# LLNL/parelagmc

Hardware: AMD Instinct MI355X
Metric: MC samples/sec (SPDE field + Darcy QoI) at stated DoF; SpMV HBM GB/s vs roofline (higher is better)
Workload: dtype f64; 1 GPU; PDESampler cube_tet r=5, 595968 DoF (n_s=196608, n_u=399360, nnz(A)=4299072), 1 MC level, corlen 0.1, SPDE field only (BASELINE config 2), 4 x 64 realizations per step, all converged; tolerance=MINRES 300 / rel 1e-6 / abs 1e-12, solver=hybridization, batch=64, streams=4, parallelism=sample-farm x1, precond_storage=fp32

## Files before the change

include/pmc.h:

```cpp
#ifndef PMC_H_
#define PMC_H_

#include <stddef.h>
#include <stdint.h>

#ifdef __cplusplus
extern "C" {
#endif

#define PMC_OK 0
#define PMC_ERR_INVALID (-1)
#define PMC_ERR_DEVICE (-2)
#define PMC_ERR_COMM (-3)
#define PMC_ERR_INTERNAL (-4)

enum pmc_memspace { PMC_MEM_HOST = 0, PMC_MEM_DEVICE = 1 };
enum pmc_projection { PMC_PROJ_NONE = 0, PMC_PROJ_GATHER = 1, PMC_PROJ_L2 = 2 };
enum pmc_storage { PMC_STORAGE_FP32 = 0, PMC_STORAGE_FP64 = 1 };

typedef struct pmc_ctx pmc_ctx;
typedef struct pmc_sampler pmc_sampler;
typedef struct pmc_darcy pmc_darcy;

typedef struct pmc_csr {
// ... 2 lines not shown
    const int32_t* colind;
    const double* vals;
} pmc_csr;

typedef struct pmc_solver_opts {
    int32_t abi_version;
    int32_t max_iter;
    double rel_tol;
    double abs_tol;
    int32_t cheb_degree_M;
    double cheb_ratio_M;
    int32_t mg_smooth_degree;
    double mg_smooth_ratio;
    int32_t mg_coarse_degree;
    double mg_coarse_ratio;
    int32_t check_every;
    int32_t use_graph;
    double schur_scale;
    int32_t mg_coarsening;
    int32_t mini_max_rows;
    int32_t two_streams;
    int32_t precond_storage;
} pmc_solver_opts;

typedef struct pmc_stats {
    int32_t iterations;
    int32_t converged;
    double initial_norm;
    double final_norm;
    double solve_ms;
    double setup_ms;
} pmc_stats;

typedef struct pmc_sampler_level {
    int32_t n_u, n_s;
    pmc_csr M;
    pmc_csr B;
    const double* w_diag;
    pmc_csr P;
} pmc_sampler_level;

typedef struct pmc_hybrid_level {
    int32_t n_lambda, n_s;
    pmc_csr H;
    pmc_csr G;
    const double* z_diag;
    const double* w_diag;
    pmc_csr P;
} pmc_hybrid_level;

typedef struct pmc_hybrid_elements {
    int32_t n_u, n_s;
    pmc_csr M_pattern;
    const int32_t* c_ptr;
    const int32_t* c_elem;
    const double* c_val;
    pmc_csr B;
    const double* w_diag;
    pmc_csr P;
} pmc_hybrid_elements;
typedef struct pmc_hybrid_system pmc_hybrid_system;

typedef struct pmc_darcy_level {
    int32_t n_u, n_p;
    pmc_csr M_pattern;
    const int32_t* c_ptr;
    const int32_t* c_elem;
    const double* c_val;
    pmc_csr B;
    const double* rhs;
    const uint8_t* ess_mask;
    const double* ess_data;
    const double* obs;
    pmc_csr P;
} pmc_darcy_level;

int pmc_version(void);
#define PMC_ABI_VERSION 3
int pmc_abi_version(void);
int pmc_krylov_z_bytes(void);
int pmc_sampler_krylov_z_bytes(const pmc_sampler* s);
int pmc_darcy_krylov_z_bytes(const pmc_darcy* d);
uint64_t pmc_kernel_launches(void);
const char* pmc_last_error(void);
void pmc_solver_opts_default(pmc_solver_opts* opts);

int pmc_ctx_create(int device_id, pmc_ctx** out);
int pmc_ctx_create_abi(int device_id, int abi_version, pmc_ctx** out);
#ifndef PMC_NO_ABI_CHECK_MACRO
#define pmc_ctx_create(device_id, out) pmc_ctx_create_abi((device_id), PMC_ABI_VERSION, (out))
#endif
void pmc_ctx_destroy(pmc_ctx* ctx);
int pmc_ctx_synchronize(pmc_ctx* ctx);
void* pmc_ctx_stream(pmc_ctx* ctx);
int pmc_ctx_device(const pmc_ctx* ctx);
int pmc_timer_start(pmc_ctx* ctx);
int pmc_timer_stop(pmc_ctx* ctx, double* ms);

int pmc_malloc(pmc_ctx* ctx, size_t bytes, void** dptr);
int pmc_free(pmc_ctx* ctx, void* dptr);
int pmc_memcpy_h2d(pmc_ctx* ctx, void* dst, const void* src, size_t bytes);
int pmc_memcpy_d2h(pmc_ctx* ctx, void* dst, const void* src, size_t bytes);

int pmc_rng_seed(pmc_ctx* ctx, uint64_t seed, int nparts, int mypart);
int pmc_normal_fill(pmc_ctx* ctx, double mean, double sigma2, uint64_t first_sample_id, uint32_t stream,
                    int nbatch, int n, double* out, int memspace);

int pmc_sampler_create(pmc_ctx* ctx, int nlevels, int n_mc_levels, const pmc_sampler_level* levels,
                       double alpha, double matern_g, int lognormal, const pmc_solver_opts* opts,
                       pmc_sampler** out);
int pmc_sampler_create_hybrid(pmc_ctx* ctx, int nlevels, const pmc_hybrid_level* levels, double alpha, double matern_g,
                              int lognormal, const pmc_solver_opts* opts, pmc_sampler** out);
int pmc_sampler_is_hybrid(const pmc_sampler* s);
int pmc_hybrid_build(const pmc_hybrid_elements* level, double alpha, pmc_hybrid_system** out);
int pmc_hybrid_system_level(const pmc_hybrid_system* sys, pmc_hybrid_level* view);
void pmc_hybrid_system_destroy(pmc_hybrid_system* sys);
int pmc_sampler_create_hybrid_from_elements(pmc_ctx* ctx, int nlevels, const pmc_hybrid_elements* levels, double alpha,
                                            double matern_g, int lognormal, const pmc_solver_opts* opts, pmc_sampler** out);
typedef struct pmc_kl_level {
    int32_t n_s;
    const double* w_diag;
    pmc_csr P;
} pmc_kl_level;
int pmc_sampler_create_kl(pmc_ctx* ctx, int nlevels, const pmc_kl_level* levels, int nmodes, const double* evals,
                          const double* evect0, int lognormal, pmc_sampler** out);
int pmc_sampler_is_kl(const pmc_sampler* s);
typedef struct pmc_kl_eigs_opts {
    double tol;
    int32_t max_iter;
    int32_t guard;
    int32_t degree;
    uint64_t seed;
} pmc_kl_eigs_opts;
typedef struct pmc_kl_eigs_info {
    int32_t iterations;
    int32_t block_products;
    int32_t converged;
    double max_residual_rel;
    double gap_rel;
    double seconds;
} pmc_kl_eigs_info;
void pmc_kl_eigs_opts_default(pmc_kl_eigs_opts* opts);
int pmc_kl_matern_apply(pmc_ctx* ctx, int dim, int n, const double* centroids, const double* w_diag, double corlen,
                        int ncols, const double* X, double* Y);
int pmc_kl_matern_eigs(pmc_ctx* ctx, int dim, int n, const double* centroids, const double* w_diag, double corlen,
                       int nmodes, const pmc_kl_eigs_opts* opts , double* evals ,
                       double* evect0 , pmc_kl_eigs_info* info );
void pmc_sampler_destroy(pmc_sampler* s);
int pmc_sampler_set_projection(pmc_sampler* s, int level, int kind, const pmc_csr* Gt,
                               const int32_t* gather_idx, const double* inv_w_orig, int orig_size);
int pmc_sampler_num_levels(const pmc_sampler* s);
int pmc_sampler_xi_size(const pmc_sampler* s, int level);
int pmc_sampler_sample_size(const pmc_sampler* s, int level);
int64_t pmc_sampler_nnz(const pmc_sampler* s, int level);
int pmc_sampler_batch_width(const pmc_sampler* s, int level);
int pmc_sampler_true_p(const pmc_sampler* s, int level, pmc_csr* out);
int pmc_sampler_sample(pmc_sampler* s, int level, uint64_t first_sample_id, int nbatch, double* xi,
                       int memspace);
int pmc_sampler_eval(pmc_sampler* s, int level, int xi_level, int nbatch, const double* xi, double* s_out,
                     const double* init_s, int init_level, int use_init, double* embed_s_out, int memspace,
                     pmc_stats* stats);

typedef struct pmc_field_stats pmc_field_stats;
int pmc_field_stats_create(pmc_sampler* s, int level, const double* chi, int memspace, pmc_field_stats** out);
void pmc_field_stats_destroy(pmc_field_stats* fs);
int pmc_field_stats_reset(pmc_field_stats* fs);
// ... 84 lines not shown
```

parelagmc_amd/capi.py:

```python
from __future__ import annotations

import ctypes as C
import weakref
import os
from typing import Optional, Sequence

import numpy as np

_HERE = os.path.dirname(os.path.abspath(__file__))
LIB_PATH = os.path.join(_HERE, "lib", "libpmc.so")

PMC_MEM_HOST, PMC_MEM_DEVICE = 0, 1
PMC_PROJ_NONE, PMC_PROJ_GATHER, PMC_PROJ_L2 = 0, 1, 2


class PmcError(RuntimeError):
    def __init__(self, code, msg):
        super().__init__(f"libpmc error {code}: {msg}")
        self.code = code


class pmc_csr(C.Structure):
    _fields_ = [("nrows", C.c_int32), ("ncols", C.c_int32), ("rowptr", C.POINTER(C.c_int32)),
                ("colind", C.POINTER(C.c_int32)), ("vals", C.POINTER(C.c_double))]


class pmc_solver_opts(C.Structure):
    _fields_ = [("abi_version", C.c_int32), ("max_iter", C.c_int32), ("rel_tol", C.c_double), ("abs_tol", C.c_double),
                ("cheb_degree_M", C.c_int32), ("cheb_ratio_M", C.c_double),
                ("mg_smooth_degree", C.c_int32), ("mg_smooth_ratio", C.c_double),
                ("mg_coarse_degree", C.c_int32), ("mg_coarse_ratio", C.c_double), ("check_every", C.c_int32),
                ("use_graph", C.c_int32), ("schur_scale", C.c_double), ("mg_coarsening", C.c_int32), ("mini_max_rows", C.c_int32),
                ("two_streams", C.c_int32), ("precond_storage", C.c_int32)]


PMC_ABI_VERSION = 3
PMC_STORAGE_FP32, PMC_STORAGE_FP64 = 0, 1


class pmc_stats(C.Structure):
    _fields_ = [("iterations", C.c_int32), ("converged", C.c_int32), ("initial_norm", C.c_double),
                ("final_norm", C.c_double), ("solve_ms", C.c_double), ("setup_ms", C.c_double)]


class pmc_sampler_level(C.Structure):
    _fields_ = [("n_u", C.c_int32), ("n_s", C.c_int32), ("M", pmc_csr), ("B", pmc_csr),
                ("w_diag", C.POINTER(C.c_double)), ("P", pmc_csr)]


class pmc_hybrid_level(C.Structure):
    _fields_ = [("n_lambda", C.c_int32), ("n_s", C.c_int32), ("H", pmc_csr), ("G", pmc_csr),
                ("z_diag", C.POINTER(C.c_double)), ("w_diag", C.POINTER(C.c_double)), ("P", pmc_csr)]


class pmc_hybrid_elements(C.Structure):
    _fields_ = [("n_u", C.c_int32), ("n_s", C.c_int32), ("M_pattern", pmc_csr), ("c_ptr", C.POINTER(C.c_int32)),
                ("c_elem", C.POINTER(C.c_int32)), ("c_val", C.POINTER(C.c_double)), ("B", pmc_csr),
                ("w_diag", C.POINTER(C.c_double)), ("P", pmc_csr)]


class pmc_kl_level(C.Structure):
    _fields_ = [("n_s", C.c_int32), ("w_diag", C.POINTER(C.c_double)), ("P", pmc_csr)]


class pmc_kl_eigs_opts(C.Structure):
    _fields_ = [("tol", C.c_double), ("max_iter", C.c_int32), ("guard", C.c_int32), ("degree", C.c_int32),
                ("seed", C.c_uint64)]


class pmc_kl_eigs_info(C.Structure):
    _fields_ = [("iterations", C.c_int32), ("block_products", C.c_int32), ("converged", C.c_int32),
                ("max_residual_rel", C.c_double), ("gap_rel", C.c_double), ("seconds", C.c_double)]


class pmc_darcy_level(C.Structure):
    _fields_ = [("n_u", C.c_int32), ("n_p", C.c_int32), ("M_pattern", pmc_csr), ("c_ptr", C.POINTER(C.c_int32)),
                ("c_elem", C.POINTER(C.c_int32)), ("c_val", C.POINTER(C.c_double)), ("B", pmc_csr),
                ("rhs", C.POINTER(C.c_double)), ("ess_mask", C.POINTER(C.c_uint8)),
                ("ess_data", C.POINTER(C.c_double)), ("obs", C.POINTER(C.c_double)), ("P", pmc_csr)]


_VP = C.c_void_p
_DP = C.c_void_p
SYMBOLS = {
    "pmc_version": (C.c_int, []),
    "pmc_last_error": (C.c_char_p, []),
    "pmc_solver_opts_default": (None, [C.POINTER(pmc_solver_opts)]),
    "pmc_abi_version": (C.c_int, []),
    "pmc_krylov_z_bytes": (C.c_int, []),
    "pmc_sampler_krylov_z_bytes": (C.c_int, [_VP]),
    "pmc_darcy_krylov_z_bytes": (C.c_int, [_VP]),
    "pmc_kernel_launches": (C.c_uint64, []),
    "pmc_ctx_create": (C.c_int, [C.c_int, C.POINTER(_VP)]),
    "pmc_ctx_create_abi": (C.c_int, [C.c_int, C.c_int, C.POINTER(_VP)]),
    "pmc_ctx_destroy": (None, [_VP]),
    "pmc_ctx_synchronize": (C.c_int, [_VP]),
    "pmc_ctx_stream": (_VP, [_VP]),
    "pmc_ctx_device": (C.c_int, [_VP]),
    "pmc_timer_start": (C.c_int, [_VP]),
    "pmc_timer_stop": (C.c_int, [_VP, C.POINTER(C.c_double)]),
    "pmc_malloc": (C.c_int, [_VP, C.c_size_t, C.POINTER(_VP)]),
    "pmc_free": (C.c_int, [_VP, _VP]),
    "pmc_memcpy_h2d": (C.c_int, [_VP, _VP, _VP, C.c_size_t]),
    "pmc_memcpy_d2h": (C.c_int, [_VP, _VP, _VP, C.c_size_t]),
    "pmc_rng_seed": (C.c_int, [_VP, C.c_uint64, C.c_int, C.c_int]),
    "pmc_normal_fill": (C.c_int, [_VP, C.c_double, C.c_double, C.c_uint64, C.c_uint32, C.c_int, C.c_int, _DP, C.c_int]),
    "pmc_sampler_create": (C.c_int, [_VP, C.c_int, C.c_int, C.POINTER(pmc_sampler_level), C.c_double, C.c_double,
                                     C.c_int, C.POINTER(pmc_solver_opts), C.POINTER(_VP)]),
    "pmc_sampler_create_hybrid": (C.c_int, [_VP, C.c_int, C.POINTER(pmc_hybrid_level), C.c_double, C.c_double, C.c_int,
                                            C.POINTER(pmc_solver_opts), C.POINTER(_VP)]),
    "pmc_sampler_is_hybrid": (C.c_int, [_VP]),
    "pmc_sampler_create_kl": (C.c_int, [_VP, C.c_int, C.POINTER(pmc_kl_level), C.c_int, C.POINTER(C.c_double),
                                        C.POINTER(C.c_double), C.c_int, C.POINTER(_VP)]),
    "pmc_sampler_is_kl": (C.c_int, [_VP]),
    "pmc_kl_eigs_opts_default": (None, [C.POINTER(pmc_kl_eigs_opts)]),
    "pmc_kl_matern_apply": (C.c_int, [_VP, C.c_int, C.c_int, C.POINTER(C.c_double), C.POINTER(C.c_double), C.c_double, C.c_int,
                                      C.POINTER(C.c_double), C.POINTER(C.c_double)]),
    "pmc_kl_matern_eigs": (C.c_int, [_VP, C.c_int, C.c_int, C.POINTER(C.c_double), C.POINTER(C.c_double), C.c_double, C.c_int,
                                     C.POINTER(pmc_kl_eigs_opts), C.POINTER(C.c_double), C.POINTER(C.c_double),
                                     C.POINTER(pmc_kl_eigs_info)]),
    "pmc_hybrid_build": (C.c_int, [C.POINTER(pmc_hybrid_elements), C.c_double, C.POINTER(_VP)]),
    "pmc_hybrid_system_level": (C.c_int, [_VP, C.POINTER(pmc_hybrid_level)]),
    "pmc_hybrid_system_destroy": (None, [_VP]),
    "pmc_sampler_create_hybrid_from_elements": (C.c_int, [_VP, C.c_int, C.POINTER(pmc_hybrid_elements), C.c_double, C.c_double,
                                                          C.c_int, C.POINTER(pmc_solver_opts), C.POINTER(_VP)]),
    "pmc_sampler_smoother_time": (C.c_int, [_VP, C.POINTER(C.c_double), C.POINTER(C.c_int64), C.POINTER(C.c_double)]),
    "pmc_sampler_smoother_bytes": (C.c_int, [_VP, C.c_int, C.c_int, C.POINTER(C.c_double)]),
    "pmc_sampler_vcycle_info": (C.c_int, [_VP, C.c_int, C.c_int, C.POINTER(C.c_int), C.POINTER(C.c_int64)]),
    "pmc_sampler_vcycle_level": (C.c_int, [_VP, C.c_int, C.c_int, C.POINTER(C.c_int), C.POINTER(C.c_double)]),
    "pmc_sampler_vcycle_prolongator": (C.c_int, [_VP, C.c_int, C.c_int, C.POINTER(C.c_int), C.POINTER(C.c_int),
                                                 C.POINTER(C.c_int64), C.POINTER(C.c_int32), C.POINTER(C.c_int32),
                                                 C.POINTER(C.c_double)]),
    "pmc_sampler_destroy": (None, [_VP]),
    "pmc_sampler_set_projection": (C.c_int, [_VP, C.c_int, C.c_int, C.POINTER(pmc_csr), C.POINTER(C.c_int32),
                                             C.POINTER(C.c_double), C.c_int]),
    "pmc_sampler_num_levels": (C.c_int, [_VP]),
    "pmc_sampler_xi_size": (C.c_int, [_VP, C.c_int]),
    "pmc_sampler_sample_size": (C.c_int, [_VP, C.c_int]),
    "pmc_sampler_batch_width": (C.c_int, [_VP, C.c_int]),
    "pmc_darcy_batch_width": (C.c_int, [_VP, C.c_int]),
    "pmc_darcy_set_operator_timing": (C.c_int, [_VP, C.c_int]),
    "pmc_darcy_operator_time": (C.c_int, [_VP, C.POINTER(C.c_double), C.POINTER(C.c_int64), C.POINTER(C.c_double)]),
    "pmc_darcy_operator_bytes": (C.c_int, [_VP, C.c_int, C.c_int, C.POINTER(C.c_double)]),
    "pmc_darcy_poly_time": (C.c_int, [_VP, C.POINTER(C.c_double), C.POINTER(C.c_int64), C.POINTER(C.c_double)]),
    "pmc_darcy_poly_bytes": (C.c_int, [_VP, C.c_int, C.c_int, C.POINTER(C.c_double)]),
    "pmc_sampler_nnz": (C.c_int64, [_VP, C.c_int]),
    "pmc_sampler_true_p": (C.c_int, [_VP, C.c_int, C.POINTER(pmc_csr)]),
    "pmc_sampler_sample": (C.c_int, [_VP, C.c_int, C.c_uint64, C.c_int, _DP, C.c_int]),
    "pmc_sampler_eval": (C.c_int, [_VP, C.c_int, C.c_int, C.c_int, _DP, _DP, _DP, C.c_int, C.c_int, _DP, C.c_int,
                                   C.POINTER(pmc_stats)]),
    "pmc_sampler_mult": (C.c_int, [_VP, C.c_int, C.c_int, _DP, _DP, C.c_int, C.c_int, C.POINTER(pmc_stats)]),
    "pmc_sampler_apply_preconditioner": (C.c_int, [_VP, C.c_int, C.c_int, _DP, _DP, C.c_int]),
    "pmc_sampler_apply_operator": (C.c_int, [_VP, C.c_int, C.c_int, _DP, _DP, C.c_int, C.c_int, C.POINTER(C.c_double),
                                             C.POINTER(C.c_double)]),
    "pmc_sampler_set_operator_timing": (C.c_int, [_VP, C.c_int]),
    "pmc_sampler_operator_time": (C.c_int, [_VP, C.POINTER(C.c_double), C.POINTER(C.c_int64)]),
    "pmc_sampler_operator_event_overhead": (C.c_int, [_VP, C.POINTER(C.c_double)]),
    "pmc_field_stats_create": (C.c_int, [_VP, C.c_int, _DP, C.c_int, C.POINTER(_VP)]),
    "pmc_field_stats_destroy": (None, [_VP]),
    "pmc_field_stats_reset": (C.c_int, [_VP]),
    "pmc_field_stats_accumulate": (C.c_int, [_VP, C.c_int, _DP, C.c_int]),
    "pmc_field_stats_run": (C.c_int, [_VP, C.c_uint64, C.c_int64]),
    "pmc_field_stats_read": (C.c_int, [_VP, _DP, _DP, _DP, C.POINTER(C.c_int64), C.c_int]),
    "pmc_field_stats_read_sums": (C.c_int, [_VP, _DP, C.POINTER(C.c_int64), C.c_int]),
    "pmc_field_stats_chi_dot": (C.c_int, [_VP, C.c_int, _DP, _DP, C.c_int]),
    "pmc_sampler_l2_error": (C.c_int, [_VP, C.c_int, C.c_int, _DP, C.c_double, _DP, C.c_int]),
    "pmc_sampler_max_error": (C.c_int, [_VP, C.c_int, C.c_int, _DP, C.c_double, _DP, C.c_int]),
    "pmc_sampler_set_output_hierarchy": (C.c_int, [_VP, C.c_int, C.POINTER(pmc_csr), C.POINTER(C.c_double)]),
    "pmc_darcy_create": (C.c_int, [_VP, C.c_int, C.c_int, C.POINTER(pmc_darcy_level), C.c_int,
                                   C.POINTER(pmc_solver_opts), C.POINTER(_VP)]),
    "pmc_darcy_create_hybrid": (C.c_int, [_VP, C.c_int, C.c_int, C.POINTER(pmc_darcy_level), C.c_int,
                                          C.POINTER(pmc_solver_opts), C.POINTER(_VP)]),
    "pmc_darcy_destroy": (None, [_VP]),
    "pmc_darcy_num_dofs": (C.c_int, [_VP, C.c_int]),
    "pmc_darcy_num_pressure_dofs": (C.c_int, [_VP, C.c_int]),
# ... 883 lines not shown
```

parelagmc_amd/csrc/capi.hip:

```cpp
#include <dlfcn.h>

#include <atomic>
#include <cstdlib>
#include <cstring>
#include <mutex>

#include "handles.hpp"

namespace pmc {

static thread_local std::string g_last_error;
void set_last_error(const std::string& m) { g_last_error = m; }

void Ctx::activate() const { PMC_HIP(hipSetDevice(device)); }
void Ctx::phase_mark(int i) const { PMC_HIP(hipEventRecord(ev_phase[i], stream)); }
void Ctx::phase_report(pmc_stats* stats, int nb) const {
    PMC_HIP(hipEventSynchronize(ev_phase[2]));
    float setup = 0.f, solve = 0.f;
    PMC_HIP(hipEventElapsedTime(&setup, ev_phase[0], ev_phase[1]));
    PMC_HIP(hipEventElapsedTime(&solve, ev_phase[1], ev_phase[2]));
    for (int k = 0; k < nb; ++k) {
        stats[k].setup_ms = (double)setup / nb;
        stats[k].solve_ms = (double)solve / nb;
    }
}

static std::atomic<int> g_live_ctx[64];
int Ctx::contexts_on_device(int device) { return g_live_ctx[device & 63].load(); }

Lanes Ctx::lanes(bool split) {
    if (split && !stream2) {
        PMC_HIP(hipStreamCreateWithFlags(&stream2, hipStreamNonBlocking));
        PMC_HIP(hipEventCreateWithFlags(&ev_fork, hipEventDisableTiming));
        PMC_HIP(hipEventCreateWithFlags(&ev_join, hipEventDisableTiming));
    }
    return Lanes{stream, split ? stream2 : stream, ev_fork, ev_join, split};
}

template <class F>
static int guarded(F&& f) {
    try {
        f();
        return PMC_OK;
    } catch (const Error& e) {
        set_last_error(e.what());
        return e.code;
    } catch (const std::bad_alloc&) {
        set_last_error("host allocation failed");
        return PMC_ERR_INTERNAL;
    } catch (const std::exception& e) {
        set_last_error(e.what());
        return PMC_ERR_INTERNAL;
    } catch (...) {
        set_last_error("unknown exception");
        return PMC_ERR_INTERNAL;
    }
}

struct UniqueId { char internal[128]; };
struct Rccl {
    void* lib = nullptr;
    int (*GetUniqueId)(UniqueId*) = nullptr;
    int (*CommInitRank)(void**, int, UniqueId, int) = nullptr;
    int (*AllReduce)(const void*, void*, size_t, int, int, void*, hipStream_t) = nullptr;
    int (*CommDestroy)(void*) = nullptr;
    const char* (*GetErrorString)(int) = nullptr;
};
static Rccl& rccl() {
    static Rccl r;
    static std::once_flag once;
    std::call_once(once, [] {
        const char* names[] = {"librccl.so.1", "librccl.so", "/opt/rocm/lib/librccl.so.1", "/opt/rocm/lib/librccl.so"};
        for (const char* n : names) {
            r.lib = dlopen(n, RTLD_NOW | RTLD_LOCAL);
            if (r.lib) break;
        }
        if (!r.lib) return;
        r.GetUniqueId = reinterpret_cast<decltype(r.GetUniqueId)>(dlsym(r.lib, "ncclGetUniqueId"));
        r.CommInitRank = reinterpret_cast<decltype(r.CommInitRank)>(dlsym(r.lib, "ncclCommInitRank"));
        r.AllReduce = reinterpret_cast<decltype(r.AllReduce)>(dlsym(r.lib, "ncclAllReduce"));
        r.CommDestroy = reinterpret_cast<decltype(r.CommDestroy)>(dlsym(r.lib, "ncclCommDestroy"));
        r.GetErrorString = reinterpret_cast<decltype(r.GetErrorString)>(dlsym(r.lib, "ncclGetErrorString"));
    });
    if (!r.lib || !r.GetUniqueId || !r.CommInitRank || !r.AllReduce || !r.CommDestroy)
        throw Error(PMC_ERR_COMM, "RCCL (librccl.so) could not be loaded");
    return r;
}
static void rccl_check(int rc, const char* what) {
    if (rc != 0) {
        Rccl& r = rccl();
        throw Error(PMC_ERR_COMM, std::string(what) + ": " + (r.GetErrorString ? r.GetErrorString(rc) : "RCCL error"));
    }
}

}

using namespace pmc;

extern "C" {

int pmc_version(void) { return 100; }
int pmc_abi_version(void) { return PMC_ABI_VERSION; }
int pmc_krylov_z_bytes(void) { return 4; }
uint64_t pmc_kernel_launches(void) { return kernel_launch_count(); }
const char* pmc_last_error(void) { return g_last_error.c_str(); }

static void check_abi(const pmc_solver_opts& o) {
    if (o.abi_version != PMC_ABI_VERSION)
        throw Error(PMC_ERR_INVALID, "pmc_solver_opts.abi_version is " + std::to_string(o.abi_version) + ", this library has " +
                                         std::to_string(PMC_ABI_VERSION) +
                                         ": fill the struct with pmc_solver_opts_default() of the header you compile against");
}

void pmc_solver_opts_default(pmc_solver_opts* o) {
    if (!o) return;
    o->max_iter = 300;
    o->rel_tol = 1e-6;
    o->abs_tol = 1e-12;
    o->abi_version = PMC_ABI_VERSION;
    o->cheb_degree_M = 0;
    o->cheb_ratio_M = 0.0;
    o->mg_smooth_degree = 2;
    o->mg_smooth_ratio = 8.0;
    o->mg_coarse_degree = 12;
    o->mg_coarse_ratio = 100.0;
    o->check_every = 2;
    o->schur_scale = 1.0;
    o->mg_coarsening = 2;
    o->mini_max_rows = 6000;
    o->two_streams = 0;
    o->use_graph = 0;
    o->precond_storage = PMC_STORAGE_FP32;
}

#undef pmc_ctx_create
int pmc_ctx_create(int device_id, pmc_ctx** out);
int pmc_ctx_create_abi(int device_id, int abi_version, pmc_ctx** out) {
    if (abi_version != PMC_ABI_VERSION) {
        if (out) *out = nullptr;
        set_last_error("caller was compiled against PMC_ABI_VERSION " + std::to_string(abi_version) + ", this library has " +
                       std::to_string(PMC_ABI_VERSION) + " (layout of pmc_solver_opts / pmc_stats): rebuild against include/pmc.h");
        return PMC_ERR_INVALID;
    }
    return pmc_ctx_create(device_id, out);
}
int pmc_ctx_create(int device_id, pmc_ctx** out) {
    return guarded([&] {
        PMC_REQUIRE(out != nullptr, "pmc_ctx_create: out is NULL");
        *out = nullptr;
        int ndev = 0;
        hipError_t e = hipGetDeviceCount(&ndev);
        if (e != hipSuccess || ndev == 0)
            throw Error(PMC_ERR_DEVICE, "no HIP device available (libpmc has no CPU fallback)");
        PMC_REQUIRE(device_id >= 0 && device_id < ndev, "pmc_ctx_create: device id out of range");
        std::unique_ptr<pmc_ctx> c(new pmc_ctx());
        c->device = device_id;
        PMC_HIP(hipSetDevice(device_id));
        PMC_HIP(hipStreamCreateWithFlags(&c->stream, hipStreamNonBlocking));
        PMC_HIP(hipEventCreate(&c->ev0));
        PMC_HIP(hipEventCreate(&c->ev1));
        for (hipEvent_t& e : c->ev_phase) PMC_HIP(hipEventCreate(&e));
        PMC_HIP(hipHostMalloc(reinterpret_cast<void**>(&c->h_flag), sizeof(int) * 16, hipHostMallocDefault));
        PMC_HIP(hipHostMalloc(reinterpret_cast<void**>(&c->h_scal), sizeof(double) * pmc::Ctx::kHostScratch, hipHostMallocDefault));
        g_live_ctx[device_id & 63].fetch_add(1);
        *out = c.release();
    });
}

void pmc_ctx_destroy(pmc_ctx* c) {
    if (!c) return;
    g_live_ctx[c->device & 63].fetch_sub(1);
    (void)hipSetDevice(c->device);
    if (c->nccl) {
        try { rccl().CommDestroy(c->nccl); } catch (...) {}
        c->nccl = nullptr;
    }
    if (c->stream) (void)hipStreamSynchronize(c->stream);
    if (c->stream2) (void)hipStreamSynchronize(c->stream2);
    if (c->h_flag) (void)hipHostFree(c->h_flag);
    if (c->h_scal) (void)hipHostFree(c->h_scal);
    if (c->ev0) (void)hipEventDestroy(c->ev0);
    if (c->ev1) (void)hipEventDestroy(c->ev1);
    for (hipEvent_t e : c->ev_phase)
        if (e) (void)hipEventDestroy(e);
    for (hipEvent_t e : {c->ev_fork, c->ev_join})
        if (e) (void)hipEventDestroy(e);
    if (c->stream2) (void)hipStreamDestroy(c->stream2);
// ... 681 lines not shown
```

parelagmc_amd/csrc/kernels.hip:

```cpp
#include "kernels.hpp"

#include <cstddef>
#include <cstdlib>

#include <algorithm>
#include <atomic>

namespace pmc {

#ifndef PMC_KBLOCK
#define PMC_KBLOCK 256
#endif
static constexpr int kBlock = PMC_KBLOCK;
static constexpr int kWave = 64;
#ifndef PMC_LEAN_GATHER
#define PMC_LEAN_GATHER 1
#endif
static constexpr bool kLeanGather = PMC_LEAN_GATHER != 0;
#ifndef PMC_LEAN_CS
#define PMC_LEAN_CS 1
#endif
static constexpr bool kLeanCs = PMC_LEAN_CS != 0;
#ifndef PMC_EG_LATE_COEF
#define PMC_EG_LATE_COEF 1
// ... 137 lines not shown
    }
}

typedef float pmc_f4 __attribute__((ext_vector_type(4)));
__device__ __forceinline__ void pin_gathers(RawVec<float, 4> (&xr)[8]) {
    pmc_f4 q0 = {xr[0].v[0], xr[0].v[1], xr[0].v[2], xr[0].v[3]}, q1 = {xr[1].v[0], xr[1].v[1], xr[1].v[2], xr[1].v[3]};
    pmc_f4 q2 = {xr[2].v[0], xr[2].v[1], xr[2].v[2], xr[2].v[3]}, q3 = {xr[3].v[0], xr[3].v[1], xr[3].v[2], xr[3].v[3]};
    pmc_f4 q4 = {xr[4].v[0], xr[4].v[1], xr[4].v[2], xr[4].v[3]}, q5 = {xr[5].v[0], xr[5].v[1], xr[5].v[2], xr[5].v[3]};
    pmc_f4 q6 = {xr[6].v[0], xr[6].v[1], xr[6].v[2], xr[6].v[3]}, q7 = {xr[7].v[0], xr[7].v[1], xr[7].v[2], xr[7].v[3]};
    asm volatile("" : "+v"(q0), "+v"(q1), "+v"(q2), "+v"(q3), "+v"(q4), "+v"(q5), "+v"(q6), "+v"(q7));
    const pmc_f4 q[8] = {q0, q1, q2, q3, q4, q5, q6, q7};
#pragma unroll
    for (int rs = 0; rs < 8; ++rs)
#pragma unroll
        for (int c = 0; c < 4; ++c) xr[rs].v[c] = q[rs][c];
}
template <typename XT, int C, int T>
__device__ __forceinline__ void pin_gathers(RawVec<XT, C> (&)[T]) {}
template <int R, int C>
__device__ __forceinline__ void pin_block(double (&a)[R][C]) {
    if constexpr (R == 8 && C == 2)
        asm volatile("" : "+v"(a[0][0]), "+v"(a[0][1]), "+v"(a[1][0]), "+v"(a[1][1]), "+v"(a[2][0]), "+v"(a[2][1]), "+v"(a[3][0]),
                     "+v"(a[3][1]), "+v"(a[4][0]), "+v"(a[4][1]), "+v"(a[5][0]), "+v"(a[5][1]), "+v"(a[6][0]), "+v"(a[6][1]),
                     "+v"(a[7][0]), "+v"(a[7][1]));
    else if constexpr (R == 4 && C == 4)
        asm volatile("" : "+v"(a[0][0]), "+v"(a[0][1]), "+v"(a[0][2]), "+v"(a[0][3]), "+v"(a[1][0]), "+v"(a[1][1]), "+v"(a[1][2]),
                     "+v"(a[1][3]), "+v"(a[2][0]), "+v"(a[2][1]), "+v"(a[2][2]), "+v"(a[2][3]), "+v"(a[3][0]), "+v"(a[3][1]),
                     "+v"(a[3][2]), "+v"(a[3][3]));
    else if constexpr (R == 2 && C == 4)
        asm volatile("" : "+v"(a[0][0]), "+v"(a[0][1]), "+v"(a[0][2]), "+v"(a[0][3]), "+v"(a[1][0]), "+v"(a[1][1]), "+v"(a[1][2]),
                     "+v"(a[1][3]));
}

template <bool NT, int C>
__device__ __forceinline__ void load_c_nt(const double* __restrict__ p, double (&v)[C]) {
    if constexpr (NT) {
#pragma unroll
        for (int i = 0; i < C; ++i) v[i] = __builtin_nontemporal_load(p + i);
    } else {
        load_c<C>(p, v);
    }
}
template <bool NT, int C>
__device__ __forceinline__ void load_v_nt(const double* __restrict__ p, double (&v)[C]) { load_c_nt<NT, C>(p, v); }
template <bool NT, int C>
__device__ __forceinline__ void load_v_nt(const float* __restrict__ p, double (&v)[C]) {
    if constexpr (NT) {
#pragma unroll
        for (int i = 0; i < C; ++i) v[i] = (double)__builtin_nontemporal_load(p + i);
    } else {
        load_cf<C>(p, v);
    }
}
template <bool NT, int C>
__device__ __forceinline__ void store_c_nt(double* __restrict__ p, const double (&v)[C]) {
    if constexpr (NT) {
#pragma unroll
        for (int i = 0; i < C; ++i) __builtin_nontemporal_store(v[i], p + i);
    } else {
        store_c<C>(p, v);
    }
}

template <bool NT, int C>
__device__ __forceinline__ void store_c_stream(double* __restrict__ p, const double (&v)[C]) {
    if constexpr (NT) {
#pragma unroll
        for (int i = 0; i < C; ++i) __builtin_nontemporal_store(v[i], p + i);
    } else {
        store_c<C>(p, v);
    }
}
template <bool NT>
__device__ __forceinline__ int load_stream(const int* __restrict__ p) {
    if constexpr (NT) return __builtin_nontemporal_load(p);
    else return *p;
}
template <bool NT>
__device__ __forceinline__ double load_stream(const double* __restrict__ p) {
    if constexpr (NT) return __builtin_nontemporal_load(p);
    else return *p;
}

template <bool NT, int C>
__device__ __forceinline__ void store_v_stream(double* __restrict__ p, const double (&v)[C]) { store_c_stream<NT, C>(p, v); }
template <bool NT, int C>
__device__ __forceinline__ void store_v_stream(float* __restrict__ p, const double (&v)[C]) {
    if constexpr (NT) {
#pragma unroll
        for (int i = 0; i < C; ++i) __builtin_nontemporal_store((float)v[i], p + i);
    } else {
        store_v<C>(p, v);
    }
}

template <int NB>
__device__ __forceinline__ void load_row(const double* __restrict__ p, double (&v)[NB]) {
    if constexpr (NB == 1) {
        v[0] = p[0];
    } else {
        const double2* q = reinterpret_cast<const double2*>(p);
#pragma unroll
        for (int i = 0; i < NB / 2; ++i) {
            double2 t = q[i];
            v[2 * i] = t.x;
            v[2 * i + 1] = t.y;
        }
    }
}
template <int NB>
__device__ __forceinline__ void store_row(double* __restrict__ p, const double (&v)[NB]) {
    if constexpr (NB == 1) {
        p[0] = v[0];
    } else {
        double2* q = reinterpret_cast<double2*>(p);
#pragma unroll
        for (int i = 0; i < NB / 2; ++i) q[i] = make_double2(v[2 * i], v[2 * i + 1]);
    }
}

__device__ __forceinline__ int vblock() { return (int)(blockIdx.z * gridDim.x + blockIdx.x); }
__device__ __forceinline__ int vgrid() { return (int)(gridDim.z * gridDim.x); }

template <int NB>
__device__ __forceinline__ void reduce_cols_store(double (&p)[Lay<NB>::C], double* __restrict__ partial, int LD = NB) {
    constexpr int C = Lay<NB>::C, T = Lay<NB>::T;
    __shared__ double lds[kBlock / kWave][NB];
#pragma unroll
    for (int c = 0; c < C; ++c) {
        double v = p[c];
#pragma unroll
        for (int off = kWave / 2; off >= T; off >>= 1) v += __shfl_xor(v, off, kWave);
        p[c] = v;
    }
    const int lane = threadIdx.x & (kWave - 1), wave = threadIdx.x / kWave;
    if (lane < T) {
#pragma unroll
        for (int c = 0; c < C; ++c) lds[wave][lane * C + c] = p[c];
    }
    __syncthreads();
    if (threadIdx.x < NB) {
        double s = 0.0;
#pragma unroll
        for (int w = 0; w < kBlock / kWave; ++w) s += lds[w][threadIdx.x];
        partial[(size_t)vblock() * LD + threadIdx.x] = s;
    }
}

__device__ __forceinline__ void reduce_cols_store_wide(const double (&p)[4], double* __restrict__ partial, int W) {
    __shared__ double lds[kBlock * 4];
#pragma unroll
    for (int c = 0; c < 4; ++c) lds[threadIdx.x * 4 + c] = p[c];
    __syncthreads();
    if ((int)threadIdx.x < W) {
        double s = 0.0;
        for (int m = threadIdx.x; m < kBlock * 4; m += W) s += lds[m];
        partial[(size_t)blockIdx.x * W + threadIdx.x] = s;
    }
}
template <int NB>
__device__ __forceinline__ void reduce_flat_store(double (&p)[Lay<NB>::C], double* __restrict__ partial, int W) {
    if constexpr (NB == kGroup) {
        if (W > NB) {
            reduce_cols_store_wide(p, partial, W);
            return;
        }
// ... 107 lines not shown
                        for (int c = 0; c < C; ++c) pdot[c] = fma((double)xr[rs].v[c], acc[rs][c], pdot[c]);
                } else if (xlast) {
#pragma unroll
                    for (int rs = 0; rs < T; ++rs)
#pragma unroll
                        for (int c = 0; c < C; ++c) xlast[rs][c] = (double)xr[rs].v[c];
                }
            }
            cj = cn;
            vj = vn;
        }
        return;
    }
    for (int j = 0; j < width; ++j, slot += kWave) {
        int cn = cj;
        double vn = vj;
        if (j + 1 < width) {
            cn = load_stream<NT>(cols + slot + kWave);
            if constexpr (!BV) vn = load_stream<NT>(vals + slot + kWave);
        }
        int cc[T];
        double aa[T];
#pragma unroll
        for (int rs = 0; rs < T; ++rs) {
            const int src = rs * G + g;
            cc[rs] = (T == 1) ? cj : __shfl(cj, src, kWave);
            if constexpr (!BV) aa[rs] = (T == 1) ? vj : __shfl(vj, src, kWave);
        }
        double xv[T][C];
        double av[T][C];
        double sv[T][C];
        if constexpr (T > 1) __builtin_amdgcn_sched_barrier(0);
#pragma unroll
        for (int rs = 0; rs < T; ++rs) {
            load_v<C>(x + (size_t)cc[rs] * LD + t * C, xv[rs]);
            if constexpr (CS) load_c<C>(cs + (size_t)cc[rs] * LD + t * C, sv[rs]);
            if constexpr (BV) load_bv<BV, C>(vals, (size_t)(slot - lane + rs * G + g) * LD + t * C, av[rs]);
        }
        if constexpr (T > 1) __builtin_amdgcn_sched_barrier(0);
#pragma unroll
        for (int rs = 0; rs < T; ++rs) {
#pragma unroll
            for (int c = 0; c < C; ++c) {
                if constexpr (CS) xv[rs][c] *= sv[rs][c];
                if constexpr (BV) acc[rs][c] = fma(av[rs][c], xv[rs][c], acc[rs][c]);
                else acc[rs][c] = fma(aa[rs], xv[rs][c], acc[rs][c]);
            }
        }
        if (xlast && j + 1 == width) {
#pragma unroll
            for (int rs = 0; rs < T; ++rs)
#pragma unroll
                for (int c = 0; c < C; ++c) xlast[rs][c] = xv[rs][c];
        }
        cj = cn;
        vj = vn;
    }
}

template <int NB, int BV, typename XT = double>
__device__ __forceinline__ void sell_row_product(const int* __restrict__ slice_off, const int* __restrict__ cols,
                                                 const double* __restrict__ vals, const XT* __restrict__ x,
                                                 int slice, int lane, int LD, double (&acc)[Lay<NB>::T][Lay<NB>::C]) {
    const int off = slice_off[slice];
    const int width = (slice_off[slice + 1] - off) >> 6;
    sell_row_range<NB, BV, false, true, false, XT>(cols, vals, x, nullptr, off, width, lane, LD, acc);
}

struct SliceWalk {
    int begin, end, stride;
};
__device__ __forceinline__ SliceWalk slice_walk(int nslices) {
    constexpr int WPB = kBlock / kWave;
    const int nblk = vgrid(), bid = vblock(), wave = threadIdx.x / kWave;
    if (nblk < 8) return SliceWalk{bid * WPB + wave, nslices, nblk * WPB};
    const int xcd = bid % 8, idx = bid / 8;
    const int nb_x = nblk / 8 + (xcd < nblk % 8 ? 1 : 0);
    const int per = (nslices + 7) / 8;
    const int lo = min(xcd * per, nslices), hi = min(lo + per, nslices);
    return SliceWalk{lo + idx * WPB + wave, hi, nb_x * WPB};
}

template <int NB, int BV, int MODE, bool DOT, int TAG, bool NT = false, bool R8 = false, bool DL = false, typename XT = double,
          typename YT = double>
__global__ __launch_bounds__(kBlock, (NB >= 32 && BV == 0 && sizeof(XT) == 4 ? 3 : 1)) void sell_spmm_kernel(int nrows, int nslices, const int* __restrict__ slice_off,
                                                           const int* __restrict__ sched,
                                                           const int* __restrict__ cols,
                                                           const double* __restrict__ vals,
                                                           const XT* __restrict__ x, typename ident<YT>::type* __restrict__ y,
                                                           const double* __restrict__ r,
                                                           const typename ident<XT>::type* __restrict__ dot_with,
                                                           double* __restrict__ partial, int ld) {
    static_assert(!R8 || (MODE == 2 && !DOT), "fused restriction goes with the residual");
    static_assert(sizeof(YT) == 8 || (MODE == 0 && !DOT && !NT), "fp32 result: plain products only");
    const int LD = row_ld<NB>(ld);
    {
        const int c0 = col0<NB>();
        x += c0;
        y += c0;
        if constexpr (BV) vals = shift_bv<BV>(vals, c0);
        if constexpr (MODE == 2) r += c0;
        if constexpr (DOT && !DL) dot_with += c0;
        if constexpr (DOT || R8) partial += c0;
    }
    static_assert(!DL || (DOT && !BV && Lay<NB>::T > 1), "diagonal-last serves the fused <x, Ax> of shared-value operators");
    constexpr int C = Lay<NB>::C, T = Lay<NB>::T, G = Lay<NB>::G;
    const int lane = threadIdx.x & (kWave - 1);
    const int g = lane / T, t = lane % T;
    double p[C];
#pragma unroll
    for (int c = 0; c < C; ++c) p[c] = 0.0;
    const SliceWalk sw = slice_walk(nslices);
    for (int si = sw.begin; si < sw.end; si += sw.stride) {
        const int slice = sched ? sched[si] : si;
        double acc[T][C];
        constexpr bool LEAN_DL = DL && lean_range<NB>();
        double xd[DL && !LEAN_DL ? T : 1][C];
        if constexpr (LEAN_DL) {
            const int off = slice_off[slice];
            sell_row_range<NB, false, false, true, NT, XT>(cols, vals, x, nullptr, off, (slice_off[slice + 1] - off) >> 6,
                                                             lane, LD, acc, nullptr, p);
        } else if constexpr (DL) {
            const int off = slice_off[slice];
            sell_row_range<NB, false, false, true, NT, XT>(cols, vals, x, nullptr, off, (slice_off[slice + 1] - off) >> 6,
                                                             lane, LD, acc, xd);
        } else if constexpr (NT) {
            const int off = slice_off[slice];
            sell_row_range<NB, BV, false, true, true, XT>(cols, vals, x, nullptr, off, (slice_off[slice + 1] - off) >> 6, lane, LD, acc);
        } else {
            sell_row_product<NB, BV, XT>(slice_off, cols, vals, x, slice, lane, LD, acc);
        }
#pragma unroll
        for (int rs = 0; rs < T; ++rs) {
            const int row = slice * kWave + rs * G + g;
            if (row < nrows) {
                const size_t at = (size_t)row * LD + t * C;
                if constexpr (MODE == 1) {
                    double old[C];
                    load_c<C>(y + at, old);
#pragma unroll
                    for (int c = 0; c < C; ++c) acc[rs][c] += old[c];
                } else if constexpr (MODE == 2) {
                    double rv[C];
                    load_c<C>(r + at, rv);
#pragma unroll
                    for (int c = 0; c < C; ++c) acc[rs][c] = rv[c] - acc[rs][c];
                }
                if constexpr (sizeof(YT) == 8) store_c_stream<NT, C>(y + at, acc[rs]);
                else store_v<C>(y + at, acc[rs]);
                if constexpr (LEAN_DL) {
                } else if constexpr (DL) {
#pragma unroll
                    for (int c = 0; c < C; ++c) p[c] = fma(xd[rs][c], acc[rs][c], p[c]);
                } else if constexpr (DOT) {
                    double w[C];
                    load_v<C>(dot_with + at, w);
#pragma unroll
                    for (int c = 0; c < C; ++c) p[c] = fma(w[c], acc[rs][c], p[c]);
                }
            } else if constexpr (R8) {
#pragma unroll
                for (int c = 0; c < C; ++c) acc[rs][c] = 0.0;
            }
            if constexpr (R8) {
                double s[C];
#pragma unroll
                for (int c = 0; c < C; ++c) {
                    double v = acc[rs][c];
                    v += __shfl_xor(v, T, kWave);
                    v += __shfl_xor(v, 2 * T, kWave);
                    v += __shfl_xor(v, 4 * T, kWave);
                    s[c] = v;
                }
                if ((g & 7) == 0 && row < nrows) store_c<C>(partial + (size_t)(row >> 3) * LD + t * C, s);
            }
        }
    }
    if constexpr (DOT) reduce_cols_store<NB>(p, partial, LD);
}

template <int NB, int BV, bool DOT, typename OT = double>
__global__ __launch_bounds__(kBlock) void sell_cheb_kernel(int nrows, int nslices, const int* __restrict__ slice_off,
                                                           const int* __restrict__ sched,
                                                           const int* __restrict__ cols,
                                                           const double* __restrict__ vals,
                                                           const double* __restrict__ dinv,
                                                           const double* __restrict__ r,
                                                           const double* __restrict__ xin, double* __restrict__ d,
                                                           OT* __restrict__ xout, double a, double b,
                                                           double* __restrict__ partial, int ld) {
    constexpr int C = Lay<NB>::C, T = Lay<NB>::T, G = Lay<NB>::G;
    const int LD = row_ld<NB>(ld);
    {
        const int c0 = col0<NB>();
        r += c0; xin += c0; d += c0; xout += c0;
        if constexpr (BV) { vals = shift_bv<BV>(vals, c0); dinv += c0; }
        if constexpr (DOT) partial += c0;
    }
    const int lane = threadIdx.x & (kWave - 1);
    const int g = lane / T, t = lane % T;
    double p[C];
#pragma unroll
    for (int c = 0; c < C; ++c) p[c] = 0.0;
    const SliceWalk sw = slice_walk(nslices);
    for (int si = sw.begin; si < sw.end; si += sw.stride) {
        const int slice = sched ? sched[si] : si;
        double acc[T][C];
        sell_row_product<NB, BV>(slice_off, cols, vals, xin, slice, lane, LD, acc);
#pragma unroll
        for (int rs = 0; rs < T; ++rs) {
            const int row = slice * kWave + rs * G + g;
            if (row >= nrows) continue;
            const size_t at = (size_t)row * LD + t * C;
            double rv[C], dv[C], xv[C], di[C];
            load_c<C>(r + at, rv);
            load_c<C>(xin + at, xv);
            if (a != 0.0) {
                load_c<C>(d + at, dv);
            } else {
#pragma unroll
                for (int c = 0; c < C; ++c) dv[c] = 0.0;
            }
            if constexpr (BV) {
                load_c<C>(dinv + at, di);
            } else {
                const double s = dinv[row];
#pragma unroll
                for (int c = 0; c < C; ++c) di[c] = s;
            }
#pragma unroll
            for (int c = 0; c < C; ++c) {
// ... 808 lines not shown
    load_c<C>(w1 + e, w1v);
    load_c<C>(x + e, xv);
#pragma unroll
    for (int c = 0; c < C; ++c) {
        w0v[c] = c0[k0 + c] * uv[c] + c1[k0 + c] * w0v[c] + c2[k0 + c] * w1v[c];
        xv[c] += c3[k0 + c] * w0v[c];
    }
    store_c<C>(w0 + e, w0v);
    store_c<C>(x + e, xv);
}

template <int NB, bool BV, bool DOT>
__global__ __launch_bounds__(kBlock) void cheb_first_kernel(size_t nflat, const double* __restrict__ dinv,
                                                            const double* __restrict__ r, double* __restrict__ d,
                                                            double* __restrict__ x, double b,
                                                            double* __restrict__ partial, int ld) {
    constexpr int C = Lay<NB>::C;
    const int W = row_ld<NB>(ld);
    double p[C];
#pragma unroll
    for (int c = 0; c < C; ++c) p[c] = 0.0;
    for (size_t i = (size_t)blockIdx.x * kBlock + threadIdx.x; i < nflat; i += (size_t)gridDim.x * kBlock) {
        const size_t e = i * C;
        double rv[C], di[C], xv[C];
        load_c<C>(r + e, rv);
        if constexpr (BV) {
            load_c<C>(dinv + e, di);
        } else {
            const double s = dinv[e / W];
#pragma unroll
            for (int c = 0; c < C; ++c) di[c] = s;
        }
#pragma unroll
        for (int c = 0; c < C; ++c) {
            xv[c] = b * di[c] * rv[c];
            if constexpr (DOT) p[c] = fma(rv[c], xv[c], p[c]);
        }
        store_c<C>(d + e, xv);
        store_c<C>(x + e, xv);
    }
    if constexpr (DOT) reduce_flat_store<NB>(p, partial, W);
}

template <int NB, typename BT = double>
__global__ __launch_bounds__(kBlock) void dot_kernel(size_t nflat, const double* __restrict__ a,
                                                     const BT* __restrict__ b, double* __restrict__ partial, int ld) {
    constexpr int C = Lay<NB>::C;
    double p[C];
#pragma unroll
    for (int c = 0; c < C; ++c) p[c] = 0.0;
    for (size_t i = (size_t)blockIdx.x * kBlock + threadIdx.x; i < nflat; i += (size_t)gridDim.x * kBlock) {
        double av[C], bv[C];
        load_c<C>(a + i * C, av);
        load_v<C>(b + i * C, bv);
#pragma unroll
        for (int c = 0; c < C; ++c) p[c] = fma(av[c], bv[c], p[c]);
    }
    reduce_flat_store<NB>(p, partial, row_ld<NB>(ld));
}

template <int NB, bool DOT, typename OT>
__global__ __launch_bounds__(kBlock) void convert_dot_kernel(size_t nflat, const double* __restrict__ in,
                                                             OT* __restrict__ out, const double* __restrict__ r,
                                                             double* __restrict__ partial, int ld) {
    constexpr int C = Lay<NB>::C;
    double p[C];
#pragma unroll
    for (int c = 0; c < C; ++c) p[c] = 0.0;
    for (size_t i = (size_t)blockIdx.x * kBlock + threadIdx.x; i < nflat; i += (size_t)gridDim.x * kBlock) {
        double v[C];
        load_c<C>(in + i * C, v);
        round_to<OT>(v);
        if constexpr (DOT) {
            double rv[C];
            load_c<C>(r + i * C, rv);
#pragma unroll
            for (int c = 0; c < C; ++c) p[c] = fma(rv[c], v[c], p[c]);
        }
        store_v<C>(out + i * C, v);
    }
    if constexpr (DOT) reduce_flat_store<NB>(p, partial, row_ld<NB>(ld));
}

template <int NB, bool NT = false>
__global__ __launch_bounds__(kBlock) void lincomb3_kernel(size_t nflat, const double* __restrict__ c0,
                                                          const double* __restrict__ a, const double* __restrict__ c1,
                                                          const double* __restrict__ b, const double* __restrict__ c2,
                                                          double* __restrict__ y, int ld, float* __restrict__ y32 = nullptr) {
    constexpr int C = Lay<NB>::C;
    const size_t i = (size_t)blockIdx.x * kBlock + threadIdx.x;
    if (i >= nflat) return;
    const size_t e = i * C;
    const int k0 = (int)(e % row_ld<NB>(ld));
    double av[C], bv[C], yv[C];
    load_c_nt<NT, C>(a + e, av);
    load_c_nt<NT, C>(b + e, bv);
    load_c_nt<NT, C>(y + e, yv);
#pragma unroll
    for (int c = 0; c < C; ++c) yv[c] = c0[k0 + c] * av[c] + c1[k0 + c] * bv[c] + c2[k0 + c] * yv[c];
    store_c<C>(y + e, yv);
    if (y32) store_v<C>(y32 + e, yv);
}

template <int NB, bool NT, typename UT>
__global__ __launch_bounds__(kBlock) void minres_wx_kernel(size_t nflat, const double* __restrict__ c0,
                                                           const UT* __restrict__ u, const double* __restrict__ c1,
                                                           double* __restrict__ w0, const double* __restrict__ c2,
                                                           const double* __restrict__ w1, const double* __restrict__ c3,
                                                           double* __restrict__ x, int ld) {
    constexpr int C = Lay<NB>::C;
    const size_t i = (size_t)blockIdx.x * kBlock + threadIdx.x;
    if (i >= nflat) return;
    const size_t e = i * C;
    const int k0 = (int)(e % row_ld<NB>(ld));
    double uv[C], w0v[C], w1v[C], xv[C];
    load_v_nt<NT, C>(u + e, uv);
    load_c_nt<NT, C>(w0 + e, w0v);
    load_c_nt<NT, C>(w1 + e, w1v);
    load_c_nt<NT, C>(x + e, xv);
#pragma unroll
    for (int c = 0; c < C; ++c) {
        w0v[c] = c0[k0 + c] * uv[c] + c1[k0 + c] * w0v[c] + c2[k0 + c] * w1v[c];
        xv[c] += c3[k0 + c] * w0v[c];
    }
    store_c_nt<NT, C>(w0 + e, w0v);
    store_c_nt<NT, C>(x + e, xv);
}

template <bool NT, typename UT, int C>
__device__ __forceinline__ void load_raw_nt(const UT* __restrict__ p, RawVec<UT, C>& r) {
    if constexpr (NT) {
#pragma unroll
        for (int i = 0; i < C; ++i) r.v[i] = __builtin_nontemporal_load(p + i);
    } else {
        load_raw<C>(p, r);
    }
}

template <int NB, bool NT, typename UT>
__global__ __launch_bounds__(kBlock) void minres_wx_deferred_kernel(size_t nflat, k::WxDeferred B,
                                                                    const double* __restrict__ cW, double* __restrict__ w0,
                                                                    double* __restrict__ w1, double* __restrict__ x, int ld) {
    constexpr int C = Lay<NB>::C;
    const size_t i = (size_t)blockIdx.x * kBlock + threadIdx.x;
    if (i >= nflat) return;
    const size_t e = i * C;
    const int k0 = (int)(e % row_ld<NB>(ld));
    double a[C], b[C], xv[C];
    if (B.first) {
#pragma unroll
        for (int c = 0; c < C; ++c) a[c] = b[c] = 0.0;
    } else {
        load_c_nt<NT, C>(w0 + e, a);
        load_c_nt<NT, C>(w1 + e, b);
    }
    if (B.first && B.x_zero) {
#pragma unroll
        for (int c = 0; c < C; ++c) xv[c] = 0.0;
    } else {
        load_c_nt<NT, C>(x + e, xv);
    }
    for (int t = 0; t < B.cnt; t += k::kWxDefer) {
        RawVec<UT, C> uv[k::kWxDefer];
#pragma unroll
        for (int j = 0; j < k::kWxDefer; ++j)
            if (t + j < B.cnt) load_raw_nt<NT>(static_cast<const UT*>(B.u[t + j]) + e, uv[j]);
#pragma unroll
        for (int j = 0; j < k::kWxDefer; ++j) {
            if (t + j < B.cnt) {
                const double* cj = cW + (size_t)B.slot[t + j] * 4 * kMaxBatch + k0;
#pragma unroll
                for (int c = 0; c < C; ++c) {
                    const double wn = cj[c] * (double)uv[j].v[c] + cj[kMaxBatch + c] * a[c] + cj[2 * kMaxBatch + c] * b[c];
                    xv[c] += cj[3 * kMaxBatch + c] * wn;
                    a[c] = b[c];
                    b[c] = wn;
                }
            }
        }
    }
    if (!B.last) {
        store_c_nt<NT, C>(w0 + e, a);
// ... 938 lines not shown
        case 4: { constexpr int NB = 4; __VA_ARGS__; } break;             \
        case 8: { constexpr int NB = 8; __VA_ARGS__; } break;             \
        case 16: { constexpr int NB = 16; __VA_ARGS__; } break;           \
        case 32: case 64: case 128: case 256: { constexpr int NB = 32; __VA_ARGS__; } break;    \
        default: throw Error(PMC_ERR_INTERNAL, "unsupported batch width"); \
    }

#define PMC_DISPATCH_NARROW(nb, ...)                                      \
    switch (nb) {                                                         \
        case 1: { constexpr int NB = 1; __VA_ARGS__; } break;             \
        case 2: { constexpr int NB = 2; __VA_ARGS__; } break;             \
        case 4: { constexpr int NB = 4; __VA_ARGS__; } break;             \
        case 8: { constexpr int NB = 8; __VA_ARGS__; } break;             \
        default: throw Error(PMC_ERR_INTERNAL, "row-split level kernels serve launches of 1, 2, 4 or 8 realizations"); \
    }

static inline dim3 groups(dim3 g, int nb) { return dim3(g.x, nb > kGroup ? (unsigned)(nb / kGroup) : 1u); }
static inline bool xcd_layout(dim3 g, int nb) {
    static const bool on = [] { const char* e = lab_env("PMC_XCD_GROUPS"); return e && atoi(e) != 0; }();
    return on && nb > kGroup && g.x >= 16;
}
static inline dim3 groups_xcd(dim3 g, int nb) {
    if (!xcd_layout(g, nb)) return groups(g, nb);
    return dim3(8u, (unsigned)(nb / kGroup), (g.x + 7u) / 8u);
}
static inline int dot_blocks(dim3 g, int nb) { return xcd_layout(g, nb) ? (int)((g.x + 7u) / 8u * 8u) : (int)g.x; }
static inline dim3 groups(unsigned g, int nb) { return groups(dim3(g), nb); }
static inline dim3 groups(int g, int nb) { return groups(dim3((unsigned)g), nb); }
static inline dim3 grid_rows(int n) { return dim3((unsigned)((n + kBlock - 1) / kBlock)); }
static inline dim3 grid_slices(int nslices) { return dim3((unsigned)((nslices + kBlock / kWave - 1) / (kBlock / kWave))); }
static inline int lay_c(int nb) { return nb >= 32 ? 4 : (nb >= 2 ? 2 : 1); }
static inline size_t flat_count(int n, int nb) { return (size_t)n * nb / lay_c(nb); }
static inline dim3 grid_flat(int n, int nb) { return dim3((unsigned)((flat_count(n, nb) + kBlock - 1) / kBlock)); }
static std::atomic<uint64_t> g_kernel_launches{0};
uint64_t kernel_launch_count() { return g_kernel_launches.load(std::memory_order_relaxed); }
void count_kernel_launches(int n) { g_kernel_launches.fetch_add((uint64_t)n, std::memory_order_relaxed); }
static inline void check_launch(int n = 1) {
    PMC_HIP(hipGetLastError());
    count_kernel_launches(n);
}
static inline void check_offsets32(const SellView& A, int nb) {
    if ((uint64_t)std::max(A.nrows, A.ncols_hint) * (uint64_t)nb >= (1ull << 32))
        throw Error(PMC_ERR_INVALID, "operand exceeds the 32-bit gather offsets of the SpMM kernels (rows x batch width >= 2^32)");
}
static inline bool nt_flat(size_t doubles) {
    static const double limit = [] {
        const char* e = lab_env("PMC_NT_FLAT_MB");
        return (e ? atof(e) : 8.0) * 1024.0 * 1024.0;
    }();
    return limit > 0.0 && (double)doubles * 8.0 > limit;
}

static unsigned dot_grid_bound() {
    static const unsigned v = [] {
        const char* e = lab_env("PMC_DOT_GRID");
        const long x = e ? atol(e) : 0;
        return x >= 8 ? (unsigned)x : 4096u;
    }();
    return v;
}

namespace k {

static inline dim3 grid_bounded(dim3 g, bool bounded) { return bounded ? dim3(std::min(g.x, dot_grid_bound())) : g; }

static inline bool nt_streams(const SellView& A, int nb, bool in_loop) {
    const double bytes = 12.0 * (double)A.nslices * 64.0 * 6.0 + 16.0 * nb * (double)A.nrows;
    static const double loop_limit = [] {
        const char* e = lab_env("PMC_NT_MIN_MB");
        return (e ? atof(e) : 128.0) * 1024.0 * 1024.0;
    }();
    return bytes > (in_loop ? loop_limit : 256.0 * 1024.0 * 1024.0);
}

static inline bool nt_poly(const SellView& A, int nb) {
    static const double limit = [] {
        const char* e = lab_env("PMC_NT_POLY_MB");
        return (e ? atof(e) : 32.0) * 1024.0 * 1024.0;
    }();
    const double bytes = 12.0 * (double)A.nslices * 64.0 * 6.0 + 16.0 * nb * (double)A.nrows;
    return limit > 0.0 && bytes > limit;
}

template <int NB, int TAG, typename XT>
static void spmm_launch(hipStream_t st, int nb, dim3 g, const SellView& A, const XT* x, double* y, bool accumulate,
                        double* dot_partial, const XT* dot_with) {
    const bool dl = TAG == 1 && Lay<NB>::T > 1 && A.diag_last && dot_with == x;
    if constexpr (!std::is_same<XT, double>::value) {
        if (A.bv || accumulate) throw Error(PMC_ERR_INTERNAL, "spmm: fp32 input with per-realization values / accumulation");
        const bool nt = TAG != 0 && nt_streams(A, NB, dot_partial != nullptr);
        if (nt) {
            if (dot_partial && dl)
                sell_spmm_kernel<NB, false, 0, true, TAG, true, false, (Lay<NB>::T > 1), XT><<<groups_xcd(g, nb), kBlock, 0, st>>>(A.nrows, A.nslices, A.slice_off, A.sched, A.cols, A.vals, x, y, nullptr, dot_with, dot_partial, nb);
            else if (dot_partial)
                sell_spmm_kernel<NB, false, 0, true, TAG, true, false, false, XT><<<groups_xcd(g, nb), kBlock, 0, st>>>(A.nrows, A.nslices, A.slice_off, A.sched, A.cols, A.vals, x, y, nullptr, dot_with, dot_partial, nb);
            else
                sell_spmm_kernel<NB, false, 0, false, TAG, true, false, false, XT><<<groups_xcd(g, nb), kBlock, 0, st>>>(A.nrows, A.nslices, A.slice_off, A.sched, A.cols, A.vals, x, y, nullptr, nullptr, nullptr, nb);
        } else {
            if (dot_partial && dl)
                sell_spmm_kernel<NB, false, 0, true, TAG, false, false, (Lay<NB>::T > 1), XT><<<groups_xcd(g, nb), kBlock, 0, st>>>(A.nrows, A.nslices, A.slice_off, A.sched, A.cols, A.vals, x, y, nullptr, dot_with, dot_partial, nb);
            else if (dot_partial)
                sell_spmm_kernel<NB, false, 0, true, TAG, false, false, false, XT><<<groups_xcd(g, nb), kBlock, 0, st>>>(A.nrows, A.nslices, A.slice_off, A.sched, A.cols, A.vals, x, y, nullptr, dot_with, dot_partial, nb);
            else
                sell_spmm_kernel<NB, false, 0, false, TAG, false, false, false, XT><<<groups_xcd(g, nb), kBlock, 0, st>>>(A.nrows, A.nslices, A.slice_off, A.sched, A.cols, A.vals, x, y, nullptr, nullptr, nullptr, nb);
        }
        return;
    } else
    if (A.bv && A.f32) {
        if (dot_partial)
            sell_spmm_kernel<NB, 2, 0, true, TAG><<<groups_xcd(g, nb), kBlock, 0, st>>>(A.nrows, A.nslices, A.slice_off, A.sched, A.cols, A.vals, x, y, nullptr, dot_with, dot_partial, nb);
        else if (accumulate)
            sell_spmm_kernel<NB, 2, 1, false, TAG><<<groups_xcd(g, nb), kBlock, 0, st>>>(A.nrows, A.nslices, A.slice_off, A.sched, A.cols, A.vals, x, y, nullptr, nullptr, nullptr, nb);
        else
            sell_spmm_kernel<NB, 2, 0, false, TAG><<<groups_xcd(g, nb), kBlock, 0, st>>>(A.nrows, A.nslices, A.slice_off, A.sched, A.cols, A.vals, x, y, nullptr, nullptr, nullptr, nb);
    } else if (A.bv) {
        if (dot_partial)
            sell_spmm_kernel<NB, true, 0, true, TAG><<<groups_xcd(g, nb), kBlock, 0, st>>>(A.nrows, A.nslices, A.slice_off, A.sched, A.cols, A.vals, x, y, nullptr, dot_with, dot_partial, nb);
        else if (accumulate)
            sell_spmm_kernel<NB, true, 1, false, TAG><<<groups_xcd(g, nb), kBlock, 0, st>>>(A.nrows, A.nslices, A.slice_off, A.sched, A.cols, A.vals, x, y, nullptr, nullptr, nullptr, nb);
        else
            sell_spmm_kernel<NB, true, 0, false, TAG><<<groups_xcd(g, nb), kBlock, 0, st>>>(A.nrows, A.nslices, A.slice_off, A.sched, A.cols, A.vals, x, y, nullptr, nullptr, nullptr, nb);
    } else if (TAG != 0 && nt_streams(A, NB, dot_partial != nullptr)) {
        if (dot_partial && dl)
            sell_spmm_kernel<NB, false, 0, true, TAG, true, false, (Lay<NB>::T > 1)><<<groups_xcd(g, nb), kBlock, 0, st>>>(A.nrows, A.nslices, A.slice_off, A.sched, A.cols, A.vals, x, y, nullptr, dot_with, dot_partial, nb);
        else if (dot_partial)
            sell_spmm_kernel<NB, false, 0, true, TAG, true><<<groups_xcd(g, nb), kBlock, 0, st>>>(A.nrows, A.nslices, A.slice_off, A.sched, A.cols, A.vals, x, y, nullptr, dot_with, dot_partial, nb);
        else if (accumulate)
            sell_spmm_kernel<NB, false, 1, false, TAG, true><<<groups_xcd(g, nb), kBlock, 0, st>>>(A.nrows, A.nslices, A.slice_off, A.sched, A.cols, A.vals, x, y, nullptr, nullptr, nullptr, nb);
        else
            sell_spmm_kernel<NB, false, 0, false, TAG, true><<<groups_xcd(g, nb), kBlock, 0, st>>>(A.nrows, A.nslices, A.slice_off, A.sched, A.cols, A.vals, x, y, nullptr, nullptr, nullptr, nb);
    } else {
        if (dot_partial && dl)
            sell_spmm_kernel<NB, false, 0, true, TAG, false, false, (Lay<NB>::T > 1)><<<groups_xcd(g, nb), kBlock, 0, st>>>(A.nrows, A.nslices, A.slice_off, A.sched, A.cols, A.vals, x, y, nullptr, dot_with, dot_partial, nb);
        else if (dot_partial)
            sell_spmm_kernel<NB, false, 0, true, TAG><<<groups_xcd(g, nb), kBlock, 0, st>>>(A.nrows, A.nslices, A.slice_off, A.sched, A.cols, A.vals, x, y, nullptr, dot_with, dot_partial, nb);
        else if (accumulate)
            sell_spmm_kernel<NB, false, 1, false, TAG><<<groups_xcd(g, nb), kBlock, 0, st>>>(A.nrows, A.nslices, A.slice_off, A.sched, A.cols, A.vals, x, y, nullptr, nullptr, nullptr, nb);
        else
            sell_spmm_kernel<NB, false, 0, false, TAG><<<groups_xcd(g, nb), kBlock, 0, st>>>(A.nrows, A.nslices, A.slice_off, A.sched, A.cols, A.vals, x, y, nullptr, nullptr, nullptr, nb);
    }
}

template <typename XT>
static int spmm_t(hipStream_t st, int nb, const SellView& A, const XT* x, double* y, bool accumulate, double* dot_partial,
                  const XT* dot_with) {
    check_offsets32(A, nb);
    if (A.nrows == 0) return 0;
    if (dot_partial && !dot_with) throw Error(PMC_ERR_INTERNAL, "spmm: fused dot without its second vector");
    dim3 g = grid_bounded(grid_slices(A.nslices), dot_partial != nullptr);
    const bool two_stage = dot_partial && A.tag != 0 && !A.bv && grid_slices(A.nslices).x > g.x;
    double* kernel_partial = dot_partial;
    if (two_stage) {
        g = grid_slices(A.nslices);
        kernel_partial = dot_partial + (size_t)kCompressBlocks * nb;
    }
    PMC_DISPATCH_NB(nb, {
        if (A.tag == 1) spmm_launch<NB, 1, XT>(st, nb, g, A, x, y, accumulate, kernel_partial, dot_with);
        else if (A.tag == 2) spmm_launch<NB, 2, XT>(st, nb, g, A, x, y, accumulate, kernel_partial, dot_with);
        else spmm_launch<NB, 0, XT>(st, nb, g, A, x, y, accumulate, kernel_partial, dot_with);
    });
    check_launch();
    if (two_stage) {
        compress_partials_kernel<<<kCompressBlocks, 256, 0, st>>>(kernel_partial, dot_blocks(g, nb), nb, dot_partial);
        check_launch();
        return kCompressBlocks;
    }
    return dot_partial ? dot_blocks(g, nb) : 0;
}
int spmm(hipStream_t st, int nb, const SellView& A, const double* x, double* y, bool accumulate, double* dot_partial,
         const double* dot_with) {
    return spmm_t<double>(st, nb, A, x, y, accumulate, dot_partial, dot_with);
}
int spmm_z(hipStream_t st, int nb, const SellView& A, zvec x, double* y, double* dot_partial, zvec dot_with) {
    if (x.f32) return spmm_t<float>(st, nb, A, x.as<float>(), y, false, dot_partial, dot_with.as<float>());
    return spmm_t<double>(st, nb, A, x.as<double>(), y, false, dot_partial, dot_with.as<double>());
}

void residual_restrict8(hipStream_t st, int nb, const SellView& A, const double* r, const double* x, double* out,
                        double* coarse) {
    check_offsets32(A, nb);
    if (A.nrows == 0) return;
    if (A.nrows % 8 != 0) throw Error(PMC_ERR_INTERNAL, "residual_restrict8: rows are not groups of 8");
    const dim3 g = grid_slices(A.nslices);
    PMC_DISPATCH_NB(nb, {
        if (A.bv && A.f32)
            sell_spmm_kernel<NB, 2, 2, false, 0, false, true><<<groups_xcd(g, nb), kBlock, 0, st>>>(A.nrows, A.nslices, A.slice_off, A.sched, A.cols, A.vals, x, out, r, nullptr, coarse, nb);
        else if (A.bv)
            sell_spmm_kernel<NB, true, 2, false, 0, false, true><<<groups_xcd(g, nb), kBlock, 0, st>>>(A.nrows, A.nslices, A.slice_off, A.sched, A.cols, A.vals, x, out, r, nullptr, coarse, nb);
        else
            sell_spmm_kernel<NB, false, 2, false, 0, false, true><<<groups_xcd(g, nb), kBlock, 0, st>>>(A.nrows, A.nslices, A.slice_off, A.sched, A.cols, A.vals, x, out, r, nullptr, coarse, nb);
    });
    check_launch();
}

void residual(hipStream_t st, int nb, const SellView& A, const double* r, const double* x, double* out) {
    check_offsets32(A, nb);
    if (A.nrows == 0) return;
    const dim3 g = grid_slices(A.nslices);
    PMC_DISPATCH_NB(nb, {
        if (A.bv && A.f32)
            sell_spmm_kernel<NB, 2, 2, false, 0><<<groups_xcd(g, nb), kBlock, 0, st>>>(A.nrows, A.nslices, A.slice_off, A.sched, A.cols, A.vals, x, out, r, nullptr, nullptr, nb);
        else if (A.bv)
            sell_spmm_kernel<NB, true, 2, false, 0><<<groups_xcd(g, nb), kBlock, 0, st>>>(A.nrows, A.nslices, A.slice_off, A.sched, A.cols, A.vals, x, out, r, nullptr, nullptr, nb);
        else
            sell_spmm_kernel<NB, false, 2, false, 0><<<groups_xcd(g, nb), kBlock, 0, st>>>(A.nrows, A.nslices, A.slice_off, A.sched, A.cols, A.vals, x, out, r, nullptr, nullptr, nb);
    });
    check_launch();
}

template <typename OT>
static int cheb_step_t(hipStream_t st, int nb, const SellView& A, const double* dinv, bool dinv_bv, const double* r,
                       const double* xin, double* d, OT* xout, double a, double b, double* dot_partial) {
    check_offsets32(A, nb);
    if (A.nrows == 0) return 0;
    if (A.bv != dinv_bv) throw Error(PMC_ERR_INTERNAL, "cheb_step: value/diagonal batching mismatch");
    const dim3 g = grid_bounded(grid_slices(A.nslices), dot_partial != nullptr);
    PMC_DISPATCH_NB(nb, {
        if (A.bv && A.f32) {
            if (dot_partial)
                sell_cheb_kernel<NB, 2, true, OT><<<groups_xcd(g, nb), kBlock, 0, st>>>(A.nrows, A.nslices, A.slice_off, A.sched, A.cols, A.vals, dinv, r, xin, d, xout, a, b, dot_partial, nb);
            else
                sell_cheb_kernel<NB, 2, false, OT><<<groups_xcd(g, nb), kBlock, 0, st>>>(A.nrows, A.nslices, A.slice_off, A.sched, A.cols, A.vals, dinv, r, xin, d, xout, a, b, nullptr, nb);
        } else if (A.bv) {
            if (dot_partial)
                sell_cheb_kernel<NB, 1, true, OT><<<groups_xcd(g, nb), kBlock, 0, st>>>(A.nrows, A.nslices, A.slice_off, A.sched, A.cols, A.vals, dinv, r, xin, d, xout, a, b, dot_partial, nb);
            else
                sell_cheb_kernel<NB, 1, false, OT><<<groups_xcd(g, nb), kBlock, 0, st>>>(A.nrows, A.nslices, A.slice_off, A.sched, A.cols, A.vals, dinv, r, xin, d, xout, a, b, nullptr, nb);
        } else {
            if (dot_partial)
                sell_cheb_kernel<NB, 0, true, OT><<<groups_xcd(g, nb), kBlock, 0, st>>>(A.nrows, A.nslices, A.slice_off, A.sched, A.cols, A.vals, dinv, r, xin, d, xout, a, b, dot_partial, nb);
            else
                sell_cheb_kernel<NB, 0, false, OT><<<groups_xcd(g, nb), kBlock, 0, st>>>(A.nrows, A.nslices, A.slice_off, A.sched, A.cols, A.vals, dinv, r, xin, d, xout, a, b, nullptr, nb);
        }
    });
    check_launch();
    return dot_partial ? dot_blocks(g, nb) : 0;
}

int cheb_step(hipStream_t st, int nb, const SellView& A, const double* dinv, bool dinv_bv, const double* r,
              const double* xin, double* d, double* xout, double a, double b, double* dot_partial) {
    return cheb_step_t<double>(st, nb, A, dinv, dinv_bv, r, xin, d, xout, a, b, dot_partial);
}

int cheb_step_z(hipStream_t st, int nb, const SellView& A, const double* dinv, bool dinv_bv, const double* r,
                const double* xin, double* d, zvec zout, double a, double b, double* dot_partial) {
    if (zout.f32) return cheb_step_t<float>(st, nb, A, dinv, dinv_bv, r, xin, d, zout.as<float>(), a, b, dot_partial);
    return cheb_step_t<double>(st, nb, A, dinv, dinv_bv, r, xin, d, zout.as<double>(), a, b, dot_partial);
}

template <typename OT>
static int poly2_t(hipStream_t st, int nb, const SellView& As, const double* dinv, bool dinv_bv, const double* r, OT* xout,
                   double c0, double c1, double* dot_partial, const double* xadd, const double* dot_with, const int* padd_idx,
                   const double* padd_x) {
    check_offsets32(As, nb);
    if (As.nrows == 0) return 0;
    if (As.bv != dinv_bv) throw Error(PMC_ERR_INTERNAL, "poly2: value/diagonal batching mismatch");
    const dim3 g = grid_bounded(grid_slices(As.nslices), dot_partial != nullptr);
    PMC_DISPATCH_NB(nb, {
// ... 396 lines not shown
}

void scale_cols_bv(hipStream_t st, int nb, int64_t nslots, const int* cols, const double* vals, const double* colscale,
                   double* out) {
    if (nslots == 0) return;
    const size_t nf = (size_t)nslots * nb / lay_c(nb);
    const unsigned g = (unsigned)std::min<size_t>((nf + kBlock - 1) / kBlock, 8192);
    PMC_DISPATCH_NB(nb, { scale_cols_bv_kernel<NB><<<g, kBlock, 0, st>>>(nf, cols, vals, colscale, out, nb); });
    check_launch();
}

void scale_cols_bv32(hipStream_t st, int nb, int64_t nslots, const int* cols, const double* vals, const double* colscale,
                     float* out_scaled, float* out_vals) {
    if (nslots == 0) return;
    const size_t nf = (size_t)nslots * nb / lay_c(nb);
    const unsigned g = (unsigned)std::min<size_t>((nf + kBlock - 1) / kBlock, 8192);
    PMC_DISPATCH_NB(nb, { scale_cols_bv32_kernel<NB><<<g, kBlock, 0, st>>>(nf, cols, vals, colscale, out_scaled, out_vals, nb); });
    check_launch();
}

void minres_wx_idx(hipStream_t st, int nb, int nsel, const int* rows, const double* c0, zvec u, const double* c1,
                   double* w0, const double* c2, const double* w1, const double* c3, double* x) {
    if (nsel == 0) return;
    PMC_DISPATCH_NB(nb, {
        if (u.f32) minres_wx_idx_kernel<NB, float><<<grid_flat(nsel, nb), kBlock, 0, st>>>(flat_count(nsel, nb), rows, c0, u.as<float>(), c1, w0, c2, w1, c3, x, nb);
        else minres_wx_idx_kernel<NB, double><<<grid_flat(nsel, nb), kBlock, 0, st>>>(flat_count(nsel, nb), rows, c0, u.as<double>(), c1, w0, c2, w1, c3, x, nb);
    });
    check_launch();
}

int cheb_first(hipStream_t st, int nb, int n, const double* dinv, bool dinv_bv, const double* r, double* d, double* x,
               double b, double* dot_partial) {
    if (n == 0) return 0;
    const size_t nf = flat_count(n, nb);
    const dim3 g = grid_bounded(grid_flat(n, nb), dot_partial != nullptr);
    PMC_DISPATCH_NB(nb, {
        if (dinv_bv) {
            if (dot_partial) cheb_first_kernel<NB, true, true><<<g, kBlock, 0, st>>>(nf, dinv, r, d, x, b, dot_partial, nb);
            else cheb_first_kernel<NB, true, false><<<g, kBlock, 0, st>>>(nf, dinv, r, d, x, b, nullptr, nb);
        } else {
            if (dot_partial) cheb_first_kernel<NB, false, true><<<g, kBlock, 0, st>>>(nf, dinv, r, d, x, b, dot_partial, nb);
            else cheb_first_kernel<NB, false, false><<<g, kBlock, 0, st>>>(nf, dinv, r, d, x, b, nullptr, nb);
        }
    });
    check_launch();
    return dot_partial ? (int)g.x : 0;
}

static inline dim3 grid_dot(int n, int nb) { return dim3(std::min(grid_flat(n, nb).x, 1024u)); }

int dot(hipStream_t st, int nb, int n, const double* a, const double* b, double* partial) {
    const dim3 g = grid_dot(n, nb);
    PMC_DISPATCH_NB(nb, { dot_kernel<NB><<<g, kBlock, 0, st>>>(flat_count(n, nb), a, b, partial, nb); });
    check_launch();
    return (int)g.x;
}

int dot_z(hipStream_t st, int nb, int n, const double* a, zvec b, double* partial) {
    const dim3 g = grid_dot(n, nb);
    PMC_DISPATCH_NB(nb, {
        if (b.f32) dot_kernel<NB, float><<<g, kBlock, 0, st>>>(flat_count(n, nb), a, b.as<float>(), partial, nb);
        else dot_kernel<NB, double><<<g, kBlock, 0, st>>>(flat_count(n, nb), a, b.as<double>(), partial, nb);
    });
    check_launch();
    return (int)g.x;
}

int convert_z(hipStream_t st, int nb, int n, const double* in, zvec out, const double* r, double* dot_partial) {
    if (n == 0) return 0;
    const dim3 g = grid_dot(n, nb);
    PMC_DISPATCH_NB(nb, {
        if (out.f32) {
            if (dot_partial) convert_dot_kernel<NB, true, float><<<g, kBlock, 0, st>>>(flat_count(n, nb), in, out.as<float>(), r, dot_partial, nb);
            else convert_dot_kernel<NB, false, float><<<g, kBlock, 0, st>>>(flat_count(n, nb), in, out.as<float>(), nullptr, nullptr, nb);
        } else {
            if (dot_partial) convert_dot_kernel<NB, true, double><<<g, kBlock, 0, st>>>(flat_count(n, nb), in, out.as<double>(), r, dot_partial, nb);
            else convert_dot_kernel<NB, false, double><<<g, kBlock, 0, st>>>(flat_count(n, nb), in, out.as<double>(), nullptr, nullptr, nb);
        }
    });
    check_launch();
    return dot_partial ? (int)g.x : 0;
}

int wdot(hipStream_t st, int nb, int n, const double* w, const double* x, double* partial) {
    const dim3 g = grid_dot(n, nb);
    PMC_DISPATCH_NB(nb, { wdot_kernel<NB><<<g, kBlock, 0, st>>>(flat_count(n, nb), w, x, partial, nb); });
    check_launch();
    return (int)g.x;
}

void reduce_final(hipStream_t st, int nb, int nblocks, const double* partial, double* out) {
    reduce_final_kernel<<<1, kScalBlock, 0, st>>>(partial, nblocks, nb, out);
    check_launch();
}

void lincomb3(hipStream_t st, int nb, int n, const double* c0, const double* a, const double* c1, const double* b,
              const double* c2, double* y, float* y32) {
    static const bool nt_on = [] { const char* e = lab_env("PMC_NT_LINCOMB"); return !e || atoi(e) != 0; }();
    const bool nt = nt_on && nt_flat((size_t)n * nb);
    PMC_DISPATCH_NB(nb, {
        if (nt) lincomb3_kernel<NB, true><<<grid_flat(n, nb), kBlock, 0, st>>>(flat_count(n, nb), c0, a, c1, b, c2, y, nb, y32);
        else lincomb3_kernel<NB><<<grid_flat(n, nb), kBlock, 0, st>>>(flat_count(n, nb), c0, a, c1, b, c2, y, nb, y32);
    });
    check_launch();
}

template <typename UT>
static void minres_wx_t(hipStream_t st, int nb, int n, const double* c0, const UT* u, const double* c1, double* w0,
                        const double* c2, const double* w1, const double* c3, double* x) {
    const bool nt = nt_flat((size_t)n * nb);
    PMC_DISPATCH_NB(nb, {
        if (nt) minres_wx_kernel<NB, true, UT><<<grid_flat(n, nb), kBlock, 0, st>>>(flat_count(n, nb), c0, u, c1, w0, c2, w1, c3, x, nb);
        else minres_wx_kernel<NB, false, UT><<<grid_flat(n, nb), kBlock, 0, st>>>(flat_count(n, nb), c0, u, c1, w0, c2, w1, c3, x, nb);
    });
}
void minres_wx(hipStream_t st, int nb, int n, const double* c0, zvec u, const double* c1, double* w0,
               const double* c2, const double* w1, const double* c3, double* x) {
    if (u.f32) minres_wx_t<float>(st, nb, n, c0, u.as<float>(), c1, w0, c2, w1, c3, x);
    else minres_wx_t<double>(st, nb, n, c0, u.as<double>(), c1, w0, c2, w1, c3, x);
    check_launch();
}

void minres_wx_deferred(hipStream_t st, int nb, int n, const MinresState* s, const WxDeferred& B, double* w0, double* w1,
                        double* x) {
    if (n == 0 || B.cnt == 0) return;
    if (B.cnt < 0 || B.cnt > kWxWindow) throw Error(PMC_ERR_INTERNAL, "minres_wx_deferred: bad count");
    const double* cW = reinterpret_cast<const double*>(reinterpret_cast<const char*>(s) + offsetof(MinresState, cW));
    const bool nt = nt_flat((size_t)n * nb);
    PMC_DISPATCH_NB(nb, {
        if (B.f32) {
            if (nt) minres_wx_deferred_kernel<NB, true, float><<<grid_flat(n, nb), kBlock, 0, st>>>(flat_count(n, nb), B, cW, w0, w1, x, nb);
            else minres_wx_deferred_kernel<NB, false, float><<<grid_flat(n, nb), kBlock, 0, st>>>(flat_count(n, nb), B, cW, w0, w1, x, nb);
        } else {
            if (nt) minres_wx_deferred_kernel<NB, true, double><<<grid_flat(n, nb), kBlock, 0, st>>>(flat_count(n, nb), B, cW, w0, w1, x, nb);
            else minres_wx_deferred_kernel<NB, false, double><<<grid_flat(n, nb), kBlock, 0, st>>>(flat_count(n, nb), B, cW, w0, w1, x, nb);
        }
    });
    check_launch();
}

void fill(hipStream_t st, size_t n, double* x, double v) {
    if (n == 0) return;
    if (v == 0.0) {
        PMC_HIP(hipMemsetAsync(x, 0, n * sizeof(double), st));
        return;
    }
    const unsigned g = (unsigned)std::min<size_t>((n + kBlock - 1) / kBlock, 2048);
    fill_kernel<<<g, kBlock, 0, st>>>(n, x, v);
    check_launch();
}

__global__ __launch_bounds__(kBlock) void scale_kernel(size_t n, const double* __restrict__ in, double a, double* __restrict__ out) {
    for (size_t i = (size_t)blockIdx.x * kBlock + threadIdx.x; i < n; i += (size_t)gridDim.x * kBlock) out[i] = a * in[i];
}
void scale(hipStream_t st, size_t n, const double* in, double a, double* out) {
    if (n == 0) return;
    const unsigned g = (unsigned)std::min<size_t>((n + kBlock - 1) / kBlock, 2048);
    scale_kernel<<<g, kBlock, 0, st>>>(n, in, a, out);
    check_launch();
}

void copy(hipStream_t st, size_t n, const double* src, double* dst) {
    if (n && src != dst) PMC_HIP(hipMemcpyAsync(dst, src, n * sizeof(double), hipMemcpyDeviceToDevice, st));
}

void minres_init(hipStream_t st, int nb, MinresState* s, const DotParts& d, double rel_tol, double abs_tol, int ring) {
// ... 231 lines not shown
```

parelagmc_amd/csrc/kernels.hpp:

```cpp
#pragma once
#include "common.hpp"

namespace pmc {

struct zvec {
    void* p = nullptr;
    bool f32 = true;
    zvec() = default;
    zvec(void* p_, bool f32_) : p(p_), f32(f32_) {}
    size_t elem_bytes() const { return f32 ? 4 : 8; }
    zvec operator+(size_t elems) const { return zvec(static_cast<char*>(p) + elems * elem_bytes(), f32); }
    explicit operator bool() const { return p != nullptr; }
    template <typename T>
    T* as() const { return static_cast<T*>(p); }
};
inline zvec zconst(const double* p) { return zvec(const_cast<double*>(p), false); }
inline zvec zconst(const float* p) { return zvec(const_cast<float*>(p), true); }
struct ZBuf {
    DevBuf<float> b;
    void ensure(size_t count, bool f32) { b.ensure(f32 ? count : 2 * count); }
    zvec v(bool f32) const { return zvec(b.p, f32); }
};

struct SellView {
    int nrows = 0, nslices = 0;
    const int* slice_off = nullptr;
    const int* cols = nullptr;
    const double* vals = nullptr;
    bool bv = false;
    const int* sched = nullptr;
    int tag = 0;
    int ncols_hint = 0;
    bool diag_last = false;
    bool f32 = false;
    int split_log2 = 0;
};
inline SellView view(const Sell& S) {
    return {S.nrows, S.nslices, S.slice_off.p, S.cols.p, S.vals.p, false, S.sched.p, 0, S.ncols, S.diag_last};
}
inline SellView view_split(const Sell& S, int sl) {
    SellView v = view(S);
    v.split_log2 = sl;
    return v;
}
inline SellView view_bv(const Sell& S, const double* vals) {
    return {S.nrows, S.nslices, S.slice_off.p, S.cols.p, vals, true, S.sched.p, 0, S.ncols};
}
inline SellView view_bv32(const Sell& S, const float* vals) {
    SellView v = view_bv(S, reinterpret_cast<const double*>(vals));
    v.f32 = true;
    return v;
}

struct EgView {
    int nrows = 0, nslices = 0, gw = 0;
    const int* cols = nullptr;
    const double* w = nullptr;
    const int* e12 = nullptr;
};

int dot_capacity(int nrows, int nb);
uint64_t kernel_launch_count();
void count_kernel_launches(int n);

namespace k {

#ifndef PMC_WX_DEFER_N
#define PMC_WX_DEFER_N 8
#endif
static constexpr int kWxDefer = PMC_WX_DEFER_N;
static constexpr int kWxWindow = 32;
struct WxDeferred {
    const void* u[kWxWindow];
    int slot[kWxWindow];
    int cnt;
    bool f32;
    bool first;
    bool x_zero;
    bool last;
};

struct MinresState {
    double beta[kMaxBatch], beta_old[kMaxBatch], eta[kMaxBatch], eta0[kMaxBatch];
    double gamma0[kMaxBatch], gamma1[kMaxBatch], sigma0[kMaxBatch], sigma1[kMaxBatch];
    double goal[kMaxBatch], alpha[kMaxBatch], delta[kMaxBatch], rho2[kMaxBatch], rho3[kMaxBatch];
    double cV[3][kMaxBatch];
    int active[kMaxBatch], iters[kMaxBatch], flag[kMaxBatch];
    int n_active, it, ring;
    double cW[kWxWindow][4][kMaxBatch];
};
static constexpr size_t kMinresHeadBytes = offsetof(MinresState, cW);

int spmm(hipStream_t st, int nb, const SellView& A, const double* x, double* y, bool accumulate,
          double* dot_partial, const double* dot_with);
int spmm_z(hipStream_t st, int nb, const SellView& A, zvec x, double* y, double* dot_partial, zvec dot_with);
void residual_restrict8(hipStream_t st, int nb, const SellView& A, const double* r, const double* x, double* out,
                        double* coarse);
void residual(hipStream_t st, int nb, const SellView& A, const double* r, const double* x, double* out);
int cheb_step(hipStream_t st, int nb, const SellView& A, const double* dinv, bool dinv_bv, const double* r,
              const double* xin, double* d, double* xout, double a, double b, double* dot_partial = nullptr);
int cheb_step_z(hipStream_t st, int nb, const SellView& A, const double* dinv, bool dinv_bv, const double* r,
                const double* xin, double* d, zvec zout, double a, double b, double* dot_partial = nullptr);
int poly2(hipStream_t st, int nb, const SellView& As, const double* dinv, bool dinv_bv, const double* r, double* xout,
          double c0, double c1, double* dot_partial = nullptr, const double* xadd = nullptr,
          const double* dot_with = nullptr, const int* padd_idx = nullptr, const double* padd_x = nullptr);
int poly2_z(hipStream_t st, int nb, const SellView& As, const double* dinv, bool dinv_bv, const double* r, zvec xout,
            double c0, double c1, double* dot_partial = nullptr, const double* xadd = nullptr,
            const double* dot_with = nullptr, const int* padd_idx = nullptr, const double* padd_x = nullptr);
void vc_presmooth32(hipStream_t st, int nb, const SellView& As, const double* dinv, zvec r, float* xout, double c0, double c1);
void vc_residual_restrict8_32(hipStream_t st, int nb, const SellView& A, zvec r, const float* x, float* out, zvec coarse);
void vc_residual32(hipStream_t st, int nb, const SellView& A, zvec r, const float* x, float* out);
void vc_residual_restrict_agg32(hipStream_t st, int nb, const SellView& A, zvec r, const float* x, float* out, zvec coarse,
                                const int* seg_ptr, const int* seg_cid, const int* seg_pos);
void vc_restrict32(hipStream_t st, int nb, const SellView& Pt, const float* res, zvec coarse);
void vc_residual_coarse32(hipStream_t st, int nb, const SellView& SP, float* res, zvec xc);
int vc_postsmooth32(hipStream_t st, int nb, const SellView& As, const double* dinv, const float* res, const float* x,
                    double* xout, double c0, double c1, const double* r, const int* parent, zvec xc, double* dot_partial);
int vc_postsmooth32_z(hipStream_t st, int nb, const SellView& As, const double* dinv, const float* res, const float* x,
                      zvec xout, double c0, double c1, const double* r, const int* parent, zvec xc, double* dot_partial);
void vc_presmooth32_bv(hipStream_t st, int nb, const SellView& As, const double* dinv, const double* r, float* xout, double c0,
                       double c1);
void vc_restrict8_32_bv(hipStream_t st, int nb, const SellView& A, const double* r, const float* x, double* coarse);
void vc_prolong8_32(hipStream_t st, int nb, int n, float* x, const double* xc);
void vc_residual32_bv(hipStream_t st, int nb, const SellView& A, const double* r, const float* x, float* out);
int vc_postsmooth32_bv(hipStream_t st, int nb, const SellView& As, const double* dinv, const float* res, const float* x,
                       double* xout, double c0, double c1, const double* r, double* dot_partial);
int vc_postsmooth32_bv_z(hipStream_t st, int nb, const SellView& As, const double* dinv, const float* res, const float* x,
                         zvec xout, double c0, double c1, const double* r, double* dot_partial);
int pair_spmm(hipStream_t st, int nb, const SellView& A1, const double* x1, const SellView& A2, const double* x2, double* y,
              double* dot_partial, const double* dot_with);
int pair_spmm_z(hipStream_t st, int nb, const SellView& A1, zvec x1, const SellView& A2, zvec x2, double* y,
                double* dot_partial, zvec dot_with);
void scale_cols_bv(hipStream_t st, int nb, int64_t nslots, const int* cols, const double* vals, const double* colscale,
                   double* out);
void scale_cols_bv32(hipStream_t st, int nb, int64_t nslots, const int* cols, const double* vals, const double* colscale,
                     float* out_scaled, float* out_vals);
void minres_wx_idx(hipStream_t st, int nb, int nsel, const int* rows, const double* c0, zvec u, const double* c1,
                   double* w0, const double* c2, const double* w1, const double* c3, double* x);
int cheb_first(hipStream_t st, int nb, int n, const double* dinv, bool dinv_bv, const double* r, double* d,
               double* x, double b, double* dot_partial = nullptr);
int dot(hipStream_t st, int nb, int n, const double* a, const double* b, double* partial);
int wdot(hipStream_t st, int nb, int n, const double* w, const double* x, double* partial);
int dot_z(hipStream_t st, int nb, int n, const double* a, zvec b, double* partial);
int convert_z(hipStream_t st, int nb, int n, const double* in, zvec out, const double* r, double* dot_partial);
void reduce_final(hipStream_t st, int nb, int nblocks, const double* partial, double* out);
void lincomb3(hipStream_t st, int nb, int n, const double* c0, const double* a, const double* c1, const double* b,
              const double* c2, double* y, float* y32 = nullptr);
void minres_wx(hipStream_t st, int nb, int n, const double* c0, zvec u, const double* c1, double* w0,
               const double* c2, const double* w1, const double* c3, double* x);
void fill(hipStream_t st, size_t n, double* x, double v);
void copy(hipStream_t st, size_t n, const double* src, double* dst);
void scale(hipStream_t st, size_t n, const double* in, double a, double* out);

struct DotParts {
    const double* p1 = nullptr;
    int n1 = 0;
    const double* p2 = nullptr;
    int n2 = 0;
    int total() const { return n1 + n2; }
};
void minres_init(hipStream_t st, int nb, MinresState* s, const DotParts& d, double rel_tol, double abs_tol, int ring = 1);
void minres_wx_deferred(hipStream_t st, int nb, int n, const MinresState* s, const WxDeferred& B, double* w0, double* w1,
                        double* x);
void minres_scal1(hipStream_t st, int nb, MinresState* s, const DotParts& d);
void minres_scal2(hipStream_t st, int nb, MinresState* s, const DotParts& d);
void minres_scal21(hipStream_t st, int nb, MinresState* s, const DotParts& d2, const DotParts& d1, double* stage = nullptr);
size_t scal_stage_doubles();

void normal_fill(hipStream_t st, int n, int nbatch, uint64_t seed, uint64_t first_id, uint32_t stream, double mean,
                 double sigma, double* out, uint64_t id_stride = 1);
void interleave(hipStream_t st, int nb, int n, const double* in, const double* w, double scale, double* out,
                const int* src = nullptr);
void deinterleave(hipStream_t st, int nb, int m, const double* in, const int* idx, const double* rowscale, bool do_exp,
                  double* out);
void broadcast(hipStream_t st, int nb, int n, const double* a, double* out);

void darcy_coef(hipStream_t st, int nb, int n, const double* kfield, bool k_divides, double* coef);
void darcy_assemble(hipStream_t st, int nb, const SellView& Mp, const int* slot_src, const int* c_ptr, const int* c_elem,
                    const double* c_val, const double* coef, const unsigned char* ess, const double* ess_data,
                    const double* rhs0, double* mvals, double* diag, double* l1inv, double* rhs_bc);
int eg_pair_spmm(hipStream_t st, int nb, const EgView& M, const double* coef, const double* x1, const SellView& A2,
                 const double* x2, double* y, double* dot_partial, const double* dot_with);
int eg_pair_spmm_z(hipStream_t st, int nb, const EgView& M, const double* coef, zvec x1, const SellView& A2,
                   zvec x2, double* y, double* dot_partial, zvec dot_with);
int eg_poly2(hipStream_t st, int nb, const EgView& M, const double* coef, const double* dinv, const double* r, double* xout,
             double c0, double c1, double* dot_partial);
int eg_poly2_z(hipStream_t st, int nb, const EgView& M, const double* coef, const double* dinv, const double* r, zvec xout,
               double c0, double c1, double* dot_partial);

void gersh_scale_bv(hipStream_t st, int nb, const SellView& S, double* dinv, double* gwork);
void refresh(hipStream_t st, int nb, int64_t nslots, const int* ptr, const int* idx, const double* w, const double* src,
             bool recip, double* out);
void darcy_backsub_u(hipStream_t st, int nb, int n_u, const int* owner, const double* kappa, const double* U0, const double* ug,
                     const double* t, double* out);
void darcy_backsub_p(hipStream_t st, int nb, int n_p, const double* kappa, const double* P0, const double* zg, const double* t,
                     double* out);
void diag_inv(hipStream_t st, int nb, int n, const int* diag_slot, const double* vals, double* dinv);

}
}

namespace pmc {
struct TailLevelDev {
    int n, nslices;
    int nslots;
    const int* slice_off;
    const int* cols;
    const double* vals;
    const double* vals_scaled;
    const double* dinv;
    int p_nslices, pt_nslices;
    const int *p_off, *p_cols, *pt_off, *pt_cols;
    const double *p_vals, *pt_vals;
    double lmax;
    int last_degree;
    double last_ratio;
    int lds_off;
    const double* ainv;
};
static constexpr size_t kTailLdsDoubles = (160 * 1024 - 1024) / 8;
struct TailParams {
    int nlev, bv, smooth_degree;
    double smooth_ratio;
    TailLevelDev lev[8];
};
struct MiniSamplerParams {
    int n_u, n_s;
// ... 26 lines not shown
```

parelagmc_amd/csrc/sampler.hip:

```cpp
#include <algorithm>
#include <cmath>

#include <cstdlib>
#include <cstring>

#include "handles.hpp"

namespace pmc {

static bool diag_last_on() {
    static const bool v = [] {
        const char* e = lab_env("PMC_DIAG_LAST");
        return !e || atoi(e) != 0;
    }();
    return v;
}


HostCsr schur_host(const HostCsr& B, const HostCsr& Bt, const std::vector<double>& dM, const double* diag_add) {
    HostCsr S;
    S.nrows = S.ncols = B.nrows;
    S.rowptr.assign(B.nrows + 1, 0);
    std::vector<int> marker(B.nrows, -1);
    std::vector<std::pair<int, double>> row;
// ... 520 lines not shown
    if (use_init) {
        double* sol_s = sol.p + (size_t)n_u * nb;
        k::fill(st, (size_t)n_u * nb, sol.p, 0.0);
        if (init_level == level) {
            k::interleave(st, nb, n_s, init_d, nullptr, 1.0, sol_s);
        } else {
            double* cur = tA.p;
            double* nxt = tB.p;
            k::interleave(st, nb, lv[init_level].n_s, init_d, nullptr, 1.0, cur);
            for (int l = init_level; l > level; --l) {
                double* dst = (l - 1 == level) ? sol_s : nxt;
                k::spmm(st, nb, view(mg.L[l - 1].P), cur, dst, false, nullptr, nullptr);
                std::swap(cur, nxt);
            }
        }
        zero_guess = false;
    }
    if (stats) ctx.phase_mark(1);
    solve_system(level, nb, zero_guess, n_u, n_s, stats);
    }
    const double* sol_s = sol.p + (size_t)n_u * nb;
    if (d.proj == PMC_PROJ_NONE) {
        k::deinterleave(st, nb, n_s, sol_s, nullptr, nullptr, lognormal, s_d);
    } else if (d.proj == PMC_PROJ_GATHER) {
        k::deinterleave(st, nb, d.out_size, sol_s, d.gather.p, nullptr, lognormal, s_d);
    } else {
        k::spmm(st, nb, view(d.Gt), sol_s, tA.p, false, nullptr, nullptr);
        k::deinterleave(st, nb, d.out_size, tA.p, nullptr, d.inv_w.p, lognormal, s_d);
    }
    if (emb_d) k::deinterleave(st, nb, n_s, sol_s, nullptr, nullptr, false, emb_d);
}

void Sampler::solve_system(int level, int nb, bool zero_guess, int x_row0, int x_nrows, pmc_stats* stats) {
    hipStream_t st = ctx.stream;
    SamplerLevel& d = lv[level];
    const int n_u = d.n_u, n_s = d.n_s, n = (int)system_rows(level);
    const bool use_amg = level < (int)amg.size() && amg[level];
    Multigrid* mgp = use_amg ? amg[level].get() : &mg;
    const int mg_l0 = use_amg ? 0 : level;
    static const int mini_env = [] {
        const char* e = lab_env("PMC_MINI_MAX_ROWS");
        return e ? atoi(e) : -1;
    }();
    const int mini_max_rows = mini_env >= 0 ? mini_env : opts.mini_max_rows;
    const int degM = opts.cheb_degree_M > 0 ? opts.cheb_degree_M : (d.ratio_M > 16.0 ? 4 : 2);
    const bool mini = !hybrid && n <= mini_max_rows && degM == 2 && opts.use_graph == 0 && mgp->use_tail &&
                      mg_l0 < (int)mgp->tail.size() && mgp->tail[mg_l0].p != nullptr;
    if (mini) {
        MiniSamplerParams mp{};
        mp.n_u = n_u;
        mp.n_s = n_s;
        mp.a_off = d.A.slice_off.p; mp.a_cols = d.A.cols.p; mp.a_vals = d.A.vals.p;
        mp.m_off = d.M.slice_off.p; mp.m_cols = d.M.cols.p; mp.m_scaled = d.M_scaled.p; mp.m_dinv = d.dinvM.p;
        cheb2_coefficients(1.0, d.ratio_M, &mp.mc0, &mp.mc1);
        mp.tail = mgp->tail[mg_l0].p;
        mp.max_iter = opts.max_iter;
        mp.rel_tol = opts.rel_tol;
        mp.abs_tol = opts.abs_tol;
        mp.x_row0 = x_row0;
        mp.x_nrows = x_nrows;
        mp.scratch_per_col = (size_t)5 * n + (size_t)3 * x_nrows;
        mini_scratch.ensure(mp.scratch_per_col * nb);
        mini_stats.ensure(kMaxBatch);
        k::mini_sampler_solve(st, nb, mp, mgp->tail_lds[mg_l0], rhs.p, sol.p, zero_guess, mini_scratch.p, mini_stats.p);
        if (stats) {
            ctx.phase_mark(2);
            PMC_HIP(hipMemcpyAsync(ctx.h_scal, mini_stats.p, sizeof(pmc_stats) * nb, hipMemcpyDeviceToHost, st));
            PMC_HIP(hipStreamSynchronize(st));
            std::memcpy(stats, ctx.h_scal, sizeof(pmc_stats) * nb);
            ctx.phase_report(stats, nb);
        }
    } else {
    LinOp A;
    A.n = n;
    A.n0 = hybrid ? 0 : n_u;
    SellView Av = view(d.A);
    Av.tag = 1;
    A.apply = [Av](const Lanes& L, int nb_, const double* x, double* y, double* partial, double*) {
        return k::DotParts{partial, k::spmm(L.main, nb_, Av, x, y, false, partial, x)};
    };
    A.apply_z = [Av](const Lanes& L, int nb_, zvec x, double* y, double* partial, double*) {
        return k::DotParts{partial, k::spmm_z(L.main, nb_, Av, x, y, partial, x)};
    };
    PrecFn prec = preconditioner(level, nb, degM, mgp, mg_l0);
    work.want_r32 = hybrid && opts.precond_storage != PMC_STORAGE_FP64 && mgp->top_reads_r32(mg_l0, nb);
    if (const char* e = lab_env("PMC_R32")) work.want_r32 = work.want_r32 && atoi(e) != 0;
    work.r32_valid = false;
    mgp->smooth_timer = (hybrid && work.op_timer.on && opts.use_graph == 0) ? &vc_timer : nullptr;
    vc_timer.on = mgp->smooth_timer != nullptr;
    GraphHint hint;
    hint.key = hash_mix(hash_mix(hash_mix(0x5a, (uint64_t)level + 1), (uint64_t)nb), (uint64_t)x_row0);
    hint.sig = hash_ptr(hash_ptr(hash_ptr(mgp->signature(mg_l0), cx.p), cd.p), cx2.p);
    MinresResult res = minres_solve(ctx, nb, A, prec, rhs.p, sol.p, zero_guess, opts, work, x_row0, x_nrows, nullptr, hint);
    if (vc_timer.on) vc_timer.harvest();
    if (stats) {
        ctx.phase_mark(2);
        for (int kcol = 0; kcol < nb; ++kcol) stats[kcol] = res.col[kcol];
        ctx.phase_report(stats, nb);
    }
    }
}

PrecFn Sampler::preconditioner(int level, int nb, int degM, Multigrid* mgp, int mg_l0) {
    SamplerLevel& d = lv[level];
    const int n_u = d.n_u;
    if (hybrid) {
        (void)nb; (void)degM;
        return [=](const Lanes& L, int nb_, const double* r, zvec z, double* dot_partial, double*) {
            mgp->r32_top = work.r32_valid ? work.r32.p : nullptr;
            work.r32_valid = false;
            const int nblk = mgp->vcycle_z(L.main, nb_, mg_l0, r, z, dot_partial);
            return k::DotParts{dot_partial, nblk, nullptr, 0};
        };
    }
    const SellView Mv = view(d.M);
    const double* dinvM = d.dinvM.p;
    ChebParams cpM{degM, 1.0, d.ratio_M, d.M_scaled.p};
    if (!cheb_fused(cpM, true)) cx2.ensure((size_t)n_u * nb);
    double* cxp = cx.p;
    double* cx2p = cx2.p;
    double* cdp = cd.p;
    return [=](const Lanes& L, int nb_, const double* r, zvec z, double* dot_partial, double* dot_partial2) {
        int nblk_u = 0;
        auto m_block = [&]() {
            L.fork();
            nblk_u = cheb_apply_z(L.side(), nb_, Mv, dinvM, false, cpM, r, z, cxp, cx2p, cdp, dot_partial2);
        };
        const int nblk_s = mgp->vcycle_z(L.main, nb_, mg_l0, r + (size_t)n_u * nb_, z + (size_t)n_u * nb_, dot_partial, m_block);
        L.join();
        return k::DotParts{dot_partial, nblk_s, dot_partial2, nblk_u};
    };
}

double Sampler::smoother_bytes(int level, int nb) const {
    if (!hybrid || level < 0 || level >= n_mc || !amg[level] || amg[level]->L.size() < 2) return 0.0;
    const MgLevel& m = amg[level]->L[0];
    const double zb = opts.precond_storage == PMC_STORAGE_FP64 ? 8.0 : 4.0;
    const double cb = amg[level]->inner_f32(1, 0, nb) ? 4.0 : 8.0;
    return 12.0 * (double)m.S.nnz + 12.0 * m.n + (double)nb * ((4.0 + 4.0 + 8.0 + zb) * m.n + cb * amg[level]->L[1].n);
}

void Sampler::apply_preconditioner(int level, int nbatch, const double* r_in, double* z_out, int memspace) {
    PMC_REQUIRE(level >= 0 && level < n_mc, "apply_preconditioner: level out of range");
    PMC_REQUIRE(valid_batch(nbatch) && nbatch <= batch_width((size_t)lv[level].n_u + lv[level].n_s, false, ctx.device) && r_in != nullptr && z_out != nullptr,
                "apply_preconditioner: nbatch must be a launch width of the level");
    ctx.activate();
    hipStream_t st = ctx.stream;
    SamplerLevel& d = lv[level];
    const size_t n = system_rows(level);
    const int nb = nbatch;
    ensure(level, nb);
    DevBuf<double> stage, zi(n * nb), part((size_t)2 * dot_capacity((int)n, nb) * nb);
    const double* r_d = r_in;
    if (memspace == PMC_MEM_HOST) {
        stage.alloc(n * nb);
        PMC_HIP(hipMemcpyAsync(stage.p, r_in, sizeof(double) * n * nb, hipMemcpyHostToDevice, st));
        r_d = stage.p;
    }
    k::interleave(st, nb, (int)n, r_d, nullptr, 1.0, rhs.p, hybrid ? d.lam_new2old.p : nullptr);
    const bool use_amg = level < (int)amg.size() && amg[level];
    Multigrid* mgp = use_amg ? amg[level].get() : &mg;
    const int degM = opts.cheb_degree_M > 0 ? opts.cheb_degree_M : (d.ratio_M > 16.0 ? 4 : 2);
    PrecFn prec = preconditioner(level, nb, degM, mgp, use_amg ? 0 : level);
    prec(ctx.lanes(false), nb, rhs.p, zvec(zi.p, false), part.p, part.p + (size_t)dot_capacity((int)n, nb) * nb);
    double* out_d = memspace == PMC_MEM_HOST ? stage.p : z_out;
    k::deinterleave(st, nb, (int)n, zi.p, hybrid ? d.lam_old2new.p : nullptr, nullptr, false, out_d);
// ... 198 lines not shown
```

parelagmc_amd/csrc/solver.hip:

```cpp
#include "solver.hpp"

#include <atomic>
#include <cmath>
#include <cstddef>
#include <cstdlib>
#include <cstring>

namespace pmc {

double* cheb_apply(hipStream_t st, int nb, const SellView& A, const double* dinv, bool dinv_bv, const ChebParams& cp,
                   const double* r, double* xa, double* xb, double* d, bool zero_guess, double* dot_partial,
                   int* dot_blocks, zvec zlast) {
    if (cp.degree < 1) throw Error(PMC_ERR_INVALID, "Chebyshev degree must be >= 1");
    const double lmax = cp.lmax, lmin = cp.lmax / cp.ratio;
    const double theta = 0.5 * (lmax + lmin), delta = 0.5 * (lmax - lmin);
    const double sigma = theta / delta;
    double rho_old = 1.0 / sigma;
    if (cheb_fused(cp, zero_guess)) {
        const double rho1 = 1.0 / (2.0 * sigma - rho_old);
        const double c0 = (1.0 + rho1 * rho_old) / theta + 2.0 * rho1 / delta;
        const double c1 = 2.0 * rho1 / (delta * theta);
        SellView As = A;
        As.vals = cp.scaled_vals;
        int nblk;
// ... 304 lines not shown
    }
    const ChebParams& cp = cp_smooth;
    double* x = cheb_apply(st, nb, A, lv.dinv.p, lv.bv, cp, r, start, other, lv.d.p, true);
    double* oth = (x == start) ? other : start;
    MgLevel& lc = L[l + 1];
    lc.ensure(nb);
    if (lv.p_oct) {
        k::residual_restrict8(st, nb, A, r, x, lv.res.p, lc.r.p);
    } else {
        k::residual(st, nb, A, r, x, lv.res.p);
        k::spmm(st, nb, view(lv.Pt), lv.res.p, lc.r.p, false, nullptr, nullptr);
    }
    double* xc = cycle(st, nb, l + 1, l0, zvec(lc.r.p, false), nullptr, zvec(), nullptr, nullptr, side).as<double>();
    if (lv.has_sp && !lv.bv && cheb_fused(cp, false)) {
        k::residual(st, nb, view(lv.SP), lv.res.p, xc, lv.res.p);
        const int nblk = cheb_post_from_residual(st, nb, A, lv.dinv.p, lv.bv, cp, r, lv.res.p, x, lv.parent.p, xc,
                                                 dot_partial, ztarget);
        if (dot_blocks) *dot_blocks = dot_partial ? nblk : 0;
        return ztarget ? zvec() : zvec(x, false);
    }
    k::spmm(st, nb, view(lv.P), xc, x, true, nullptr, nullptr);
    return zvec(cheb_apply(st, nb, A, lv.dinv.p, lv.bv, cp, r, x, oth, lv.d.p, false, dot_partial, dot_blocks, ztarget), false);
}

int Multigrid::cycle_role(int l0, int nb, int l, bool* in_tail) const {
    bool tail_on = false;
    for (int q = l0; q < (int)L.size(); ++q) {
        const MgLevel& lv = L[(size_t)q];
        const bool last = q == (int)L.size() - 1 || lv.is_last;
        int role = -1;
        if (!tail_on) {
            if (q > l0 && nb <= dense_nb && lv.dense_inv.p) {
                role = 2;
            } else {
                const bool tail_later = nb <= tail_later_nb && lv.n > 4096 && !last && q + 1 < (int)tail.size() && tail[q + 1].p;
                tail_on = use_tail && q < (int)tail.size() && tail[q].p && !tail_later;
            }
        }
        if (role < 0) role = !last ? 0 : (tail_on && lv.ainv.p) ? 2 : 1;
        if (q == l) {
            if (in_tail) *in_tail = tail_on;
            return role;
        }
        if (role != 0) break;
    }
    if (in_tail) *in_tail = false;
    return 3;
}

int Multigrid::vcycle(hipStream_t st, int nb, int l0, const double* r, double* xout, double* dot_partial,
                      const std::function<void()>& side) {
    int nblk = 0;
    const zvec res = cycle(st, nb, l0, l0, zconst(r), xout, zvec(), dot_partial, &nblk, side ? &side : nullptr);
    if (res.p != xout || res.f32) throw Error(PMC_ERR_INTERNAL, "V-cycle result landed in the wrong buffer");
    return nblk;
}

int Multigrid::vcycle_z(hipStream_t st, int nb, int l0, const double* r, zvec zout, double* dot_partial,
                        const std::function<void()>& side) {
    int nblk = 0;
    cycle(st, nb, l0, l0, zconst(r), nullptr, zout, dot_partial, &nblk, side ? &side : nullptr);
    return nblk;
}

MinresWork::~MinresWork() {
    for (auto& kv : graphs)
        if (kv.second.exec) (void)hipGraphExecDestroy(kv.second.exec);
}

uint64_t Multigrid::signature(int l0) const {
    uint64_t h = 0x1234;
    for (int l = l0; l < (int)L.size(); ++l) {
        const MgLevel& m = L[l];
        h = hash_ptr(h, m.r.p); h = hash_ptr(h, m.xa.p); h = hash_ptr(h, m.xb.p); h = hash_ptr(h, m.d.p);
        h = hash_ptr(h, m.SP.vals.p); h = hash_ptr(h, m.parent.p);
        h = hash_ptr(h, m.res.p); h = hash_ptr(h, m.vals_bv.p); h = hash_ptr(h, m.vals_scaled.p); h = hash_ptr(h, m.dinv.p);
        h = hash_ptr(h, m.vals32.p); h = hash_ptr(h, m.scaled32.p);
        h = hash_ptr(h, m.vals_t.p); h = hash_ptr(h, m.scaled_t.p); h = hash_ptr(h, m.dinv_t.p);
        if (l < (int)tail.size()) h = hash_ptr(h, tail[l].p);
    }
    return h;
}

void MinresWork::ensure(int n, int nb, bool z32) {
    const size_t need = (size_t)n * nb;
    v0.ensure(need); v1.ensure(need); u0.ensure(need, z32); u1.ensure(need, z32);
    w0.ensure(need); w1.ensure(need); q.ensure(need);
    partial.ensure((size_t)2 * dot_capacity(n, nb) * nb);
    partial_op.ensure((size_t)2 * dot_capacity(n, nb) * nb);
    if (!state.p) state.alloc(1);
    stage.ensure(k::scal_stage_doubles());
}

__global__ void axpby_kernel(size_t n, double a, const double* __restrict__ x, double b, double* __restrict__ y) {
    size_t i = (size_t)blockIdx.x * blockDim.x + threadIdx.x;
    const size_t stride = (size_t)gridDim.x * blockDim.x;
    for (; i < n; i += stride) y[i] = a * x[i] + b * y[i];
}
static void axpby(hipStream_t st, size_t n, double a, const double* x, double b, double* y) {
    if (!n) return;
    const unsigned g = (unsigned)std::min<size_t>((n + 255) / 256, 4096);
    axpby_kernel<<<g, 256, 0, st>>>(n, a, x, b, y);
    PMC_HIP(hipGetLastError());
    count_kernel_launches(1);
}

static size_t split_threshold() {
    static const size_t v = [] {
        const char* e = lab_env("PMC_SPLIT_MIN");
        return e ? (size_t)atoll(e) : (size_t)1500000;
    }();
    return v;
}

static bool stage_on() {
    static const bool v = [] {
        const char* e = lab_env("PMC_SCAL_STAGE");
        return !e || atoi(e) != 0;
    }();
    return v;
}
static size_t sampler_wide_rows(int device) {
    static std::atomic<size_t> cache[64];
    const int slot = device & 63;
    size_t v = cache[slot].load(std::memory_order_relaxed);
    if (v == 0) {
        size_t total_b = 0;
        hipDevice_t dev;
        if (hipDeviceGet(&dev, device) != hipSuccess || hipDeviceTotalMem(&total_b, dev) != hipSuccess || total_b == 0)
            v = (size_t)5000000;
        else
            v = (size_t)((double)total_b * 0.5 / (110.0 * 32.0 * 8.0));
        cache[slot].store(v, std::memory_order_relaxed);
    }
    return v;
}

static size_t wx_ring_budget(int device) {
    static std::atomic<size_t> cache[64];
    const int slot = device & 63;
    size_t v = cache[slot].load(std::memory_order_relaxed);
    if (v == 0) {
        size_t total_b = 0;
        hipDevice_t dev;
        if (hipDeviceGet(&dev, device) != hipSuccess || hipDeviceTotalMem(&total_b, dev) != hipSuccess) total_b = 0;
        v = total_b / 128 + 1;
        cache[slot].store(v, std::memory_order_relaxed);
    }
    return v - 1;
}

int batch_width(size_t rows, bool darcy, int device) {
    static const auto lim = [](const char* name, size_t dflt) {
        const char* e = lab_env(name);
        return e ? (size_t)atoll(e) : dflt;
    };
    static const size_t l32 = lim("PMC_WIDE_ROWS", 300000),
                        l32s_lab = lim("PMC_S_WIDE_ROWS", lab_env("PMC_WIDE_ROWS") ? l32 : 0),
                        l64 = lim("PMC_W64_ROWS", 150000), l128 = lim("PMC_W128_ROWS", 40000), l256 = lim("PMC_W256_ROWS", 20000),
                        l64s = lim("PMC_S_W64_ROWS", lab_env("PMC_W64_ROWS") ? l64 : 700000);
    const size_t l32s = l32s_lab ? l32s_lab : (darcy ? 0 : sampler_wide_rows(device));
    if (rows > (darcy ? l32 : l32s)) return 16;
    if (rows <= l256) return 256;
    if (rows <= l128) return 128;
    if (rows <= (darcy ? l64 : l64s)) return 64;
    return 32;
}

static bool wx_defer_on() {
    static const bool v = [] {
        const char* e = lab_env("PMC_WX_DEFER");
        return !e || atoi(e) != 0;
    }();
    return v;
}

static int wx_window(int device, size_t vec_bytes) {
    static const int lab = [] {
        const char* e = lab_env("PMC_WX_WINDOW");
        return e ? std::min(std::max(atoi(e), 1), k::kWxWindow) : 0;
    }();
    if (lab) return lab;
    const size_t fit = wx_ring_budget(device) / std::max<size_t>(vec_bytes, 1);
    return (int)std::min<size_t>(std::max<size_t>(fit, 9) - 1, (size_t)k::kWxWindow);
}

static bool late_wx() {
    static const bool v = [] {
        const char* e = lab_env("PMC_LATE_WX");
        return !e || atoi(e) != 0;
    }();
    return v;
}

MinresResult minres_solve(Ctx& ctx, int nb, const LinOp& A, const PrecFn& prec, const double* b, double* x,
                          bool zero_guess, const pmc_solver_opts& o, MinresWork& w, int x_row0, int x_nrows,
                          const int* x_rows, GraphHint hint) {
    hipStream_t st = ctx.stream;
    const int n = A.n;
    const size_t len = (size_t)n * nb;
    const bool split = o.two_streams == 1 || (o.two_streams == 0 && split_threshold() > 0 && len >= split_threshold() &&
                                              Ctx::contexts_on_device(ctx.device) == 1);
    const Lanes L = ctx.lanes(split);
    const bool z32 = o.precond_storage != PMC_STORAGE_FP64;
    w.ensure(n, nb, z32);
    k::MinresState* S = w.state.p;
    double* v0 = w.v0.p; double* v1 = w.v1.p; zvec u0 = w.u0.v(z32); zvec u1 = w.u1.v(z32);
    double* w0 = w.w0.p; double* w1 = w.w1.p; double* q = w.q.p;

    if (x_rows && !zero_guess) throw Error(PMC_ERR_INTERNAL, "minres: compact solution needs a zero initial guess");
    if (!A.apply_z || (!zero_guess && !A.apply)) throw Error(PMC_ERR_INTERNAL, "minres: operator closures missing");
    if (x_row0 < 0 || x_nrows < 0 || (!x_rows && x_row0 + x_nrows > n))
        throw Error(PMC_ERR_INTERNAL, "minres: bad solution row range");
    const size_t xoff = (size_t)x_row0 * nb;
    const int every = o.check_every > 0 ? o.check_every : 1;
    const bool graphs = hint.key != 0 && o.use_graph != 0 && every == 2;
    const bool late = L.split && !graphs && A.n0 > 0 && A.n0 < n && late_wx();
    const bool defer = !graphs && !late && !x_rows && wx_defer_on();
    if (zero_guess) {
        if (defer) {
            k::fill(st, xoff, x, 0.0);
            k::fill(st, len - xoff - (size_t)x_nrows * nb, x + xoff + (size_t)x_nrows * nb, 0.0);
        } else {
            k::fill(st, x_rows ? (size_t)x_nrows * nb : len, x, 0.0);
        }
        k::copy(st, len, b, v1);
    } else {
        A.apply(L, nb, x, v1, nullptr, nullptr);
        axpby(st, len, 1.0, b, -1.0, v1);
    }
    const size_t seg2 = (size_t)dot_capacity(n, nb) * nb;
    const bool r32 = w.want_r32 && z32;
    if (r32) {
        w.r32.ensure(len);
        k::convert_z(st, nb, n, v1, zvec(reinterpret_cast<double*>(w.r32.p), true), nullptr, nullptr);
        w.r32_valid = true;
    }
    k::DotParts dp = prec(L, nb, v1, u1, w.partial.p, w.partial.p + seg2);
    if (dp.total() == 0) dp = k::DotParts{w.partial.p, k::dot_z(st, nb, n, v1, u1, w.partial.p)};
    const int window = defer ? wx_window(ctx.device, len * (z32 ? sizeof(float) : sizeof(double))) : 1;
    k::minres_init(st, nb, S, dp, o.rel_tol, o.abs_tol, window);
    k::fill(st, len, v0, 0.0);
    if (!defer) {
        k::fill(st, len, w0, 0.0);
        k::fill(st, len, w1, 0.0);
    }

    auto coef = [&](size_t off) { return reinterpret_cast<const double*>(reinterpret_cast<const char*>(S) + off); };
    const double* cV0 = coef(offsetof(k::MinresState, cV));
    const double* cV1 = cV0 + kMaxBatch;
    const double* cV2 = cV1 + kMaxBatch;
    const double* cW0 = coef(offsetof(k::MinresState, cW));
    const double* cW1 = cW0 + kMaxBatch;
    const double* cW2 = cW1 + kMaxBatch;
    const double* cW3 = cW2 + kMaxBatch;
    const int* d_nactive = reinterpret_cast<const int*>(reinterpret_cast<const char*>(S) + offsetof(k::MinresState, n_active));

    auto poll = [&]() {
        PMC_HIP(hipMemcpyAsync(ctx.h_flag, d_nactive, sizeof(int), hipMemcpyDeviceToHost, st));
        PMC_HIP(hipStreamSynchronize(st));
        return *ctx.h_flag;
    };

    MinresResult out;
    zvec u2;
    if (late) {
        w.u2.ensure(len, z32);
        u2 = w.u2.v(z32);
    }
    const bool timing = w.op_timer.on && !(hint.key != 0 && o.use_graph != 0);
    k::DotParts dp_op;
    auto apply_op = [&](zvec u) {
        if (timing) w.op_timer.begin(st);
        dp_op = A.apply_z(L, nb, u, q, w.partial_op.p, w.partial_op.p + seg2);
        if (timing) w.op_timer.end(st);
    };
    struct PendingWx { zvec u; double *w0 = nullptr, *w1 = nullptr; } pend;
    auto wx = [&](hipStream_t s, zvec u_, double* w0_, double* w1_) {
        if (x_rows) k::minres_wx_idx(s, nb, x_nrows, x_rows, cW0, u_, cW1, w0_, cW2, w1_, cW3, x);
        else k::minres_wx(s, nb, x_nrows, cW0, u_ + xoff, cW1, w0_, cW2, w1_, cW3, x + xoff);
    };
    auto flush_wx = [&](hipStream_t s) {
        if (pend.u) wx(s, pend.u, pend.w0, pend.w1);
        pend.u = zvec();
    };
    auto iteration = [&](zvec u0_, zvec u1_, double* v0_, double* v1_, double* w0_, double* w1_, bool last) {
        if (late) {
            const size_t off = (size_t)A.n0 * nb;
            L.fork();
            k::lincomb3(L.aux, nb, A.n0, cV0, q, cV1, v1_, cV2, v0_);
            flush_wx(L.aux);
            k::lincomb3(st, nb, n - A.n0, cV0, q + off, cV1, v1_ + off, cV2, v0_ + off);
        } else {
            k::lincomb3(st, nb, n, cV0, q, cV1, v1_, cV2, v0_, r32 ? w.r32.p : nullptr);
            w.r32_valid = r32;
        }
        k::DotParts d2 = prec(L, nb, v0_, u0_, w.partial.p, w.partial.p + seg2);
        if (d2.total() == 0) d2 = k::DotParts{w.partial.p, k::dot_z(st, nb, n, v0_, u0_, w.partial.p)};
        if (!last) {
            apply_op(u0_);
            k::minres_scal21(st, nb, S, d2, dp_op, stage_on() ? w.stage.p : nullptr);
        } else {
            k::minres_scal2(st, nb, S, d2);
        }
        if (defer) return;
        if (late && !last) pend = PendingWx{u1_, w0_, w1_};
        else wx(st, u1_, w0_, w1_);
    };
    auto pair = [&]() {
        iteration(u0, u1, v0, v1, w0, w1, false);
        iteration(u1, u0, v1, v0, w1, w0, false);
    };
    int it = 0;
    int n_active = poll();
    const uint64_t hint_key = hint.key ? hash_mix(hint.key, zero_guess ? 1 : 2) : 0;
    int first_poll = 0;
    if (hint_key) {
        auto f = w.iter_hint.find(hint_key);
        if (f != w.iter_hint.end()) first_poll = std::max(0, f->second - 4);
    }
    const int poll_step = graphs ? 2 : every;
    const int mid_poll = first_poll >= 8 ? (first_poll / 2 / poll_step) * poll_step : -1;
    if (n_active > 0 && o.max_iter > 0) {
        apply_op(u1);
        k::minres_scal1(st, nb, S, dp_op);
    }
    if (graphs) {
        if (n_active > 0 && it + 2 <= o.max_iter) {
            pair();
            it += 2;
            n_active = poll();
        }
        if (n_active > 0 && it + 2 <= o.max_iter) {
            uint64_t sig = hash_mix(hint.sig, (uint64_t)nb);
            sig = hash_mix(sig, (uint64_t)n);
            for (const void* p : {(const void*)b, (const void*)x, (const void*)v0, (const void*)v1, (const void*)u0.p,
                                  (const void*)u1.p, (const void*)w0, (const void*)w1, (const void*)q,
                                  (const void*)w.partial.p, (const void*)w.partial_op.p, (const void*)S, (const void*)w.stage.p,
                                  (const void*)x_rows, (const void*)(r32 ? w.r32.p : nullptr)})
                sig = hash_ptr(sig, p);
            sig = hash_mix(sig, ((uint64_t)x_row0 << 32) ^ (uint64_t)x_nrows);
            sig = hash_mix(sig, L.split ? 7 : 3);
            MinresWork::GraphEntry& ge = w.graphs[hint.key];
            if (ge.exec && ge.sig != sig) {
                PMC_HIP(hipGraphExecDestroy(ge.exec));
                ge.exec = nullptr;
            }
            if (!ge.exec) {
                hipGraph_t graph = nullptr;
                PMC_HIP(hipStreamBeginCapture(st, hipStreamCaptureModeThreadLocal));
                try {
                    pair();
                } catch (...) {
                    (void)hipStreamEndCapture(st, &graph);
                    if (graph) (void)hipGraphDestroy(graph);
                    throw;
                }
                PMC_HIP(hipStreamEndCapture(st, &graph));
                PMC_HIP(hipGraphInstantiate(&ge.exec, graph, nullptr, nullptr, 0));
                PMC_HIP(hipGraphDestroy(graph));
                ge.sig = sig;
            }
            while (n_active > 0 && it + 2 <= o.max_iter) {
                PMC_HIP(hipGraphLaunch(ge.exec, st));
                it += 2;
                if (it >= first_poll || it == mid_poll) n_active = poll();
            }
        }
        if (n_active > 0 && it < o.max_iter) {
            iteration(u0, u1, v0, v1, w0, w1, true);
            ++it;
            n_active = poll();
        }
    } else if (defer) {
        zvec ub[k::kWxWindow + 1];
        ub[0] = u1;
        ub[1] = u0;
        int have = 2, c = 0;
        k::WxDeferred pending{};
        pending.f32 = z32;
        pending.first = true;
        pending.x_zero = zero_guess;
        auto flush = [&](bool last) {
            if (pending.cnt == 0) return;
            pending.last = last;
            k::minres_wx_deferred(st, nb, x_nrows, S, pending, w0, w1, x + xoff);
            pending.cnt = 0;
            pending.first = false;
            std::swap(ub[0], ub[c]);
            c = 0;
        };
        while (n_active > 0 && it < o.max_iter) {
            ++it;
            if (c + 1 == have) {
                if (w.ring.size() < (size_t)have - 1) w.ring.resize((size_t)have - 1);
                w.ring[(size_t)have - 2].ensure(len, z32);
// ... 67 lines not shown
```

parelagmc_amd/csrc/solver.hpp:

```cpp
#pragma once
#include <functional>
#include <map>
#include <vector>

#include "kernels.hpp"

namespace pmc {

struct ChebParams {
    int degree = 3;
    double lmax = 1.0;
    double ratio = 8.0;
    const double* scaled_vals = nullptr;
};
inline void cheb2_coefficients(double lmax, double ratio, double* c0, double* c1) {
    const double lmin = lmax / ratio;
    const double theta = 0.5 * (lmax + lmin), delta = 0.5 * (lmax - lmin), sigma = theta / delta;
    const double rho_old = 1.0 / sigma, rho1 = 1.0 / (2.0 * sigma - rho_old);
    *c0 = (1.0 + rho1 * rho_old) / theta + 2.0 * rho1 / delta;
    *c1 = 2.0 * rho1 / (delta * theta);
}
inline bool cheb_fused(const ChebParams& cp, bool ) { return cp.degree == 2 && cp.scaled_vals; }
double* cheb_apply(hipStream_t st, int nb, const SellView& A, const double* dinv, bool dinv_bv, const ChebParams& cp,
                   const double* r, double* xa, double* xb, double* d, bool zero_guess,
// ... 15 lines not shown
    DevBuf<double> vals_bv;
    DevBuf<double> vals_scaled;
    DevBuf<double> vals_t, scaled_t, dinv_t;
    DevBuf<float> vals32, scaled32;
    bool f32 = false;
    bool bv = false;
    double lmax = 2.0;
    bool is_last = false;
    int last_degree = 12;
    double last_ratio = 100.0;
    Sell P, Pt;
    HostCsr P_host;
    Sell SP;
    DevBuf<int> parent;
    bool has_sp = false;
    bool p_oct = false;
    bool p_agg = false;
    DevBuf<int> seg_ptr, seg_cid, seg_pos;
    DevBuf<double> r, xa, xb, d, res;
    DevBuf<double> ainv;
    DevBuf<double> dense_inv;
    int split_log2 = 0, sp_split_log2 = 0;
    Sell S_split, SP_split;
    DevBuf<double> scaled_split;
    void ensure(int nb);
    SellView sview() const { return bv ? (f32 ? view_bv32(S, vals32.p) : view_bv(S, vals_bv.p)) : view(S); }
    const double* scaled_ptr() const { return (bv && f32) ? reinterpret_cast<const double*>(scaled32.p) : vals_scaled.p; }
};

struct OpTimer;
struct Multigrid {
    std::vector<MgLevel> L;
    int smooth_degree = 2;
    double smooth_ratio = 4.0;
    int coarse_degree = 12;
    double coarse_ratio = 100.0;
    std::vector<DevBuf<TailParams>> tail;
    std::vector<size_t> tail_lds;
    bool use_tail = true;
    bool f32_intermediates = true;
    bool f32_any_injection = false;
    int tail_later_nb = 0;
    int dense_nb = 0;
    const float* r32_top = nullptr;
    bool top_reads_r32(int l0, int nb) const {
        if (l0 < 0 || l0 + 1 >= (int)L.size()) return false;
        const MgLevel& lv = L[(size_t)l0];
        const bool tail_later = nb <= tail_later_nb && lv.n > 4096 && l0 + 1 < (int)tail.size() && tail[(size_t)l0 + 1].p;
        const bool tail_here = use_tail && l0 < (int)tail.size() && tail[(size_t)l0].p && !tail_later;
        return !tail_here && !lv.is_last && !lv.bv && lv.has_sp && !lv.p_oct && f32_any_injection && smooth_degree == 2 &&
               lv.vals_scaled.p && f32_intermediates;
    }
    OpTimer* smooth_timer = nullptr;
    void build_tails(hipStream_t st);
    void enable_bv_tail(int max_rows = 8192);
    int bv_tail_width = 0;
    void ensure_bv_tail_width(hipStream_t st, int nb);
    void refresh_bv_tail(hipStream_t st, int nb, int first_level = 0);
    int cycle_role(int l0, int nb, int l, bool* in_tail) const;
    uint64_t signature(int l0) const;
    int vcycle(hipStream_t st, int nb, int l0, const double* r, double* xout, double* dot_partial = nullptr,
               const std::function<void()>& side = nullptr);
    int vcycle_z(hipStream_t st, int nb, int l0, const double* r, zvec zout, double* dot_partial = nullptr,
                 const std::function<void()>& side = nullptr);

    struct LevelPath {
        bool last = false, dense = false, tail_here = false, f32_shared = false, f32_bv = false;
    };
    LevelPath level_path(int l, int l0, int nb) const;
    bool inner_f32(int l, int l0, int nb) const;

  private:
    zvec cycle(hipStream_t st, int nb, int l, int l0, zvec rz, double* target, zvec ztarget, double* dot_partial,
               int* dot_blocks, const std::function<void()>* side);
};

struct LinOp {
    int n = 0;
    int n0 = 0;
    std::function<k::DotParts(const Lanes& L, int nb, const double* x, double* y, double* dot_partial,
                              double* dot_partial2)> apply;
    std::function<k::DotParts(const Lanes& L, int nb, zvec x, double* y, double* dot_partial,
                              double* dot_partial2)> apply_z;
};
using PrecFn = std::function<k::DotParts(const Lanes& L, int nb, const double* r, zvec z, double* dot_partial,
                                         double* dot_partial2)>;

struct GraphHint {
    uint64_t key = 0, sig = 0;
};
inline uint64_t hash_mix(uint64_t h, uint64_t v) {
    h ^= v + 0x9E3779B97F4A7C15ull + (h << 6) + (h >> 2);
    return h;
}
inline uint64_t hash_ptr(uint64_t h, const void* p) { return hash_mix(h, (uint64_t)(uintptr_t)p); }

struct OpTimer {
    bool on = false;
    std::vector<hipEvent_t> ev;
    size_t used = 0;
    double ms = 0.0, gap_ms = 0.0;
    int64_t launches = 0;
    OpTimer() = default;
    OpTimer(const OpTimer&) = delete;
    OpTimer& operator=(const OpTimer&) = delete;
    ~OpTimer() {
        for (hipEvent_t e : ev) (void)hipEventDestroy(e);
    }
    void begin(hipStream_t st) {
        while (ev.size() < used + 3) {
            hipEvent_t e;
            PMC_HIP(hipEventCreate(&e));
            ev.push_back(e);
        }
        PMC_HIP(hipEventRecord(ev[used], st));
    }
    void end(hipStream_t st) {
        PMC_HIP(hipEventRecord(ev[used + 1], st));
        PMC_HIP(hipEventRecord(ev[used + 2], st));
        used += 3;
    }
    void harvest() {
        for (size_t e = 0; e + 2 < used; e += 3) {
            float a = 0.f, g = 0.f;
            PMC_HIP(hipEventElapsedTime(&a, ev[e], ev[e + 1]));
            PMC_HIP(hipEventElapsedTime(&g, ev[e + 1], ev[e + 2]));
            ms += a;
            gap_ms += g;
            ++launches;
        }
        used = 0;
    }
    void clear() { ms = gap_ms = 0.0; launches = 0; }
};

struct MinresWork {
    DevBuf<double> v0, v1, w0, w1, q, partial;
    ZBuf u0, u1;
    DevBuf<double> stage;
    ZBuf u2;
    std::vector<ZBuf> ring;
    DevBuf<double> partial_op;
    DevBuf<float> r32;
    bool want_r32 = false, r32_valid = false;
    std::map<uint64_t, int> iter_hint;
    DevBuf<k::MinresState> state;
    struct GraphEntry {
        uint64_t sig = 0;
        hipGraphExec_t exec = nullptr;
    };
    std::map<uint64_t, GraphEntry> graphs;
    OpTimer op_timer;
    MinresWork() = default;
    MinresWork(const MinresWork&) = delete;
    MinresWork& operator=(const MinresWork&) = delete;
    ~MinresWork();
    void ensure(int n, int nb, bool z32);
};

struct MinresResult {
    pmc_stats col[kMaxBatch];
    int iterations = 0;
};

MinresResult minres_solve(Ctx& ctx, int nb, const LinOp& A, const PrecFn& prec, const double* b, double* x,
                          bool zero_guess, const pmc_solver_opts& o, MinresWork& w, int x_row0, int x_nrows,
                          const int* x_rows = nullptr, GraphHint hint = GraphHint());

double gershgorin_scaled(const HostCsr& A, const std::vector<double>& diag, double* lmin = nullptr);

}
```

Before: 4131 samples/s.

## Fuse MINRES Lanczos three-term update into a second SpMV pass

In the hybridized MINRES solver, the operator application is split into a dot-only SpMV pass that computes <u, Au> without storing Au. A second SpMV pass then recomputes Au and directly applies the Lanczos three-term combination, writing both the fp64 vector and its fp32 copy. This removes the q buffer, its write and read, and the separate lincomb3 and convert launches. The cost is a second sweep over the matrix and fp32 input per iteration. A copy kernel that also emits the fp32 residual copy replaces the initial copy-plus-convert.

```diff
diff --git a/include/pmc.h b/include/pmc.h
--- a/include/pmc.h
+++ b/include/pmc.h
@@ -108,6 +108,7 @@
 int pmc_sampler_krylov_z_bytes(const pmc_sampler* s);
 int pmc_darcy_krylov_z_bytes(const pmc_darcy* d);
 uint64_t pmc_kernel_launches(void);
+uint64_t pmc_fused_lanczos_solves(void);
 const char* pmc_last_error(void);
 void pmc_solver_opts_default(pmc_solver_opts* opts);
 
diff --git a/parelagmc_amd/capi.py b/parelagmc_amd/capi.py
--- a/parelagmc_amd/capi.py
+++ b/parelagmc_amd/capi.py
@@ -91,6 +91,7 @@
     "pmc_sampler_krylov_z_bytes": (C.c_int, [_VP]),
     "pmc_darcy_krylov_z_bytes": (C.c_int, [_VP]),
     "pmc_kernel_launches": (C.c_uint64, []),
+    "pmc_fused_lanczos_solves": (C.c_uint64, []),
     "pmc_ctx_create": (C.c_int, [C.c_int, C.POINTER(_VP)]),
     "pmc_ctx_create_abi": (C.c_int, [C.c_int, C.c_int, C.POINTER(_VP)]),
     "pmc_ctx_destroy": (None, [_VP]),
diff --git a/parelagmc_amd/csrc/capi.hip b/parelagmc_amd/csrc/capi.hip
--- a/parelagmc_amd/csrc/capi.hip
+++ b/parelagmc_amd/csrc/capi.hip
@@ -103,6 +103,7 @@
 int pmc_abi_version(void) { return PMC_ABI_VERSION; }
 int pmc_krylov_z_bytes(void) { return 4; }
 uint64_t pmc_kernel_launches(void) { return kernel_launch_count(); }
+uint64_t pmc_fused_lanczos_solves(void) { return fused_lanczos_solve_count(); }
 const char* pmc_last_error(void) { return g_last_error.c_str(); }
 
 static void check_abi(const pmc_solver_opts& o) {
diff --git a/parelagmc_amd/csrc/kernels.hip b/parelagmc_amd/csrc/kernels.hip
--- a/parelagmc_amd/csrc/kernels.hip
+++ b/parelagmc_amd/csrc/kernels.hip
@@ -243,6 +243,14 @@
     else return *p;
 }
 
+template <int C>
+__device__ __forceinline__ void lanczos_combine(const double* __restrict__ c0, const double* __restrict__ c1,
+                                                const double* __restrict__ c2, int k0, const double (&a)[C],
+                                                const double (&b)[C], double (&y)[C]) {
+#pragma unroll
+    for (int c = 0; c < C; ++c) y[c] = c0[k0 + c] * a[c] + c1[k0 + c] * b[c] + c2[k0 + c] * y[c];
+}
+
 template <bool NT, int C>
 __device__ __forceinline__ void store_v_stream(double* __restrict__ p, const double (&v)[C]) { store_c_stream<NT, C>(p, v); }
 template <bool NT, int C>
@@ -516,7 +524,7 @@
 }
 
 template <int NB, int BV, int MODE, bool DOT, int TAG, bool NT = false, bool R8 = false, bool DL = false, typename XT = double,
-          typename YT = double>
+          typename YT = double, int LZ = 0>
 __global__ __launch_bounds__(kBlock, (NB >= 32 && BV == 0 && sizeof(XT) == 4 ? 3 : 1)) void sell_spmm_kernel(int nrows, int nslices, const int* __restrict__ slice_off,
                                                            const int* __restrict__ sched,
                                                            const int* __restrict__ cols,
@@ -524,18 +532,25 @@
                                                            const XT* __restrict__ x, typename ident<YT>::type* __restrict__ y,
                                                            const double* __restrict__ r,
                                                            const typename ident<XT>::type* __restrict__ dot_with,
-                                                           double* __restrict__ partial, int ld) {
+                                                           double* __restrict__ partial, int ld,
+                                                           k::LanczosUpdate lz = k::LanczosUpdate{}) {
     static_assert(!R8 || (MODE == 2 && !DOT), "fused restriction goes with the residual");
+    static_assert(LZ == 0 || (BV == 0 && MODE == 0 && !R8 && sizeof(YT) == 8 && DOT == (LZ == 1)),
+                  "Lanczos passes: shared values, plain product; the dot-only pass has the dot, the update passes none");
     static_assert(sizeof(YT) == 8 || (MODE == 0 && !DOT && !NT), "fp32 result: plain products only");
     const int LD = row_ld<NB>(ld);
     {
         const int c0 = col0<NB>();
         x += c0;
-        y += c0;
+        if constexpr (LZ != 1) y += c0;
         if constexpr (BV) vals = shift_bv<BV>(vals, c0);
         if constexpr (MODE == 2) r += c0;
         if constexpr (DOT && !DL) dot_with += c0;
         if constexpr (DOT || R8) partial += c0;
+        if constexpr (LZ >= 2) {
+            lz.v1 += c0; lz.y32 += c0;
+            lz.c0 += c0; lz.c1 += c0; lz.c2 += c0;
+        }
     }
     static_assert(!DL || (DOT && !BV && Lay<NB>::T > 1), "diagonal-last serves the fused <x, Ax> of shared-value operators");
     constexpr int C = Lay<NB>::C, T = Lay<NB>::T, G = Lay<NB>::G;
@@ -580,7 +595,20 @@
 #pragma unroll
                     for (int c = 0; c < C; ++c) acc[rs][c] = rv[c] - acc[rs][c];
                 }
-                if constexpr (sizeof(YT) == 8) store_c_stream<NT, C>(y + at, acc[rs]);
+                if constexpr (LZ >= 2) {
+                    double bv[C], yv[C];
+                    load_c_nt<NT, C>(lz.v1 + at, bv);
+                    if constexpr (LZ == 2) {
+                        load_c_nt<NT, C>(y + at, yv);
+                    } else {
+#pragma unroll
+                        for (int c = 0; c < C; ++c) yv[c] = 0.0;
+                    }
+                    lanczos_combine<C>(lz.c0, lz.c1, lz.c2, t * C, acc[rs], bv, yv);
+                    store_c<C>(y + at, yv);
+                    store_v<C>(lz.y32 + at, yv);
+                } else if constexpr (LZ == 1) {
+                } else if constexpr (sizeof(YT) == 8) store_c_stream<NT, C>(y + at, acc[rs]);
                 else store_v<C>(y + at, acc[rs]);
                 if constexpr (LEAN_DL) {
                 } else if constexpr (DL) {
@@ -1555,6 +1583,18 @@
     if constexpr (DOT) reduce_flat_store<NB>(p, partial, row_ld<NB>(ld));
 }
 
+template <int NB>
+__global__ __launch_bounds__(kBlock) void copy_r32_kernel(size_t nflat, const double* __restrict__ in,
+                                                          double* __restrict__ out, float* __restrict__ out32) {
+    constexpr int C = Lay<NB>::C;
+    for (size_t i = (size_t)blockIdx.x * kBlock + threadIdx.x; i < nflat; i += (size_t)gridDim.x * kBlock) {
+        double v[C];
+        load_c<C>(in + i * C, v);
+        store_c<C>(out + i * C, v);
+        store_v<C>(out32 + i * C, v);
+    }
+}
+
 template <int NB, bool NT = false>
 __global__ __launch_bounds__(kBlock) void lincomb3_kernel(size_t nflat, const double* __restrict__ c0,
                                                           const double* __restrict__ a, const double* __restrict__ c1,
@@ -1569,8 +1609,7 @@
     load_c_nt<NT, C>(a + e, av);
     load_c_nt<NT, C>(b + e, bv);
     load_c_nt<NT, C>(y + e, yv);
-#pragma unroll
-    for (int c = 0; c < C; ++c) yv[c] = c0[k0 + c] * av[c] + c1[k0 + c] * bv[c] + c2[k0 + c] * yv[c];
+    lanczos_combine<C>(c0, c1, c2, k0, av, bv, yv);
     store_c<C>(y + e, yv);
     if (y32) store_v<C>(y32 + e, yv);
 }
@@ -2675,12 +2714,31 @@
     return limit > 0.0 && bytes > limit;
 }
 
+#define PMC_SPMM_LZ(NTF, DLF, LZF)                                                                                          \
+    sell_spmm_kernel<NB, false, 0, (LZF) == 1, TAG, NTF, false, DLF, XT, double, LZF><<<groups_xcd(g, nb), kBlock, 0, st>>>( \
+        A.nrows, A.nslices, A.slice_off, A.sched, A.cols, A.vals, x, y, nullptr, dot_with, dot_partial, nb, *lz)
+
 template <int NB, int TAG, typename XT>
 static void spmm_launch(hipStream_t st, int nb, dim3 g, const SellView& A, const XT* x, double* y, bool accumulate,
-                        double* dot_partial, const XT* dot_with) {
+                        double* dot_partial, const XT* dot_with, int lz_mode = 0, const LanczosUpdate* lz = nullptr) {
     const bool dl = TAG == 1 && Lay<NB>::T > 1 && A.diag_last && dot_with == x;
     if constexpr (!std::is_same<XT, double>::value) {
         if (A.bv || accumulate) throw Error(PMC_ERR_INTERNAL, "spmm: fp32 input with per-realization values / accumulation");
+        if constexpr (TAG == 1) {
+            if (lz_mode) {
+                const bool ntl = nt_streams(A, NB, true);
+                constexpr bool kDl = Lay<NB>::T > 1;
+                if (lz_mode == 1) {
+                    if (ntl) { if (dl) PMC_SPMM_LZ(true, kDl, 1); else PMC_SPMM_LZ(true, false, 1); }
+                    else { if (dl) PMC_SPMM_LZ(false, kDl, 1); else PMC_SPMM_LZ(false, false, 1); }
+                } else if (lz_mode == 2) {
+                    if (ntl) PMC_SPMM_LZ(true, false, 2); else PMC_SPMM_LZ(false, false, 2);
+                } else {
+                    if (ntl) PMC_SPMM_LZ(true, false, 3); else PMC_SPMM_LZ(false, false, 3);
+                }
+                return;
+            }
+        }
         const bool nt = TAG != 0 && nt_streams(A, NB, dot_partial != nullptr);
         if (nt) {
             if (dot_partial && dl)
@@ -2736,7 +2794,7 @@
 
 template <typename XT>
 static int spmm_t(hipStream_t st, int nb, const SellView& A, const XT* x, double* y, bool accumulate, double* dot_partial,
-                  const XT* dot_with) {
+                  const XT* dot_with, int lz_mode = 0, const LanczosUpdate* lz = nullptr) {
     check_offsets32(A, nb);
     if (A.nrows == 0) return 0;
     if (dot_partial && !dot_with) throw Error(PMC_ERR_INTERNAL, "spmm: fused dot without its second vector");
@@ -2748,7 +2806,7 @@
         kernel_partial = dot_partial + (size_t)kCompressBlocks * nb;
     }
     PMC_DISPATCH_NB(nb, {
-        if (A.tag == 1) spmm_launch<NB, 1, XT>(st, nb, g, A, x, y, accumulate, kernel_partial, dot_with);
+        if (A.tag == 1) spmm_launch<NB, 1, XT>(st, nb, g, A, x, y, accumulate, kernel_partial, dot_with, lz_mode, lz);
         else if (A.tag == 2) spmm_launch<NB, 2, XT>(st, nb, g, A, x, y, accumulate, kernel_partial, dot_with);
         else spmm_launch<NB, 0, XT>(st, nb, g, A, x, y, accumulate, kernel_partial, dot_with);
     });
@@ -2767,6 +2825,22 @@
 int spmm_z(hipStream_t st, int nb, const SellView& A, zvec x, double* y, double* dot_partial, zvec dot_with) {
     if (x.f32) return spmm_t<float>(st, nb, A, x.as<float>(), y, false, dot_partial, dot_with.as<float>());
     return spmm_t<double>(st, nb, A, x.as<double>(), y, false, dot_partial, dot_with.as<double>());
+}
+
+static void check_lanczos_pass(const SellView& A, zvec x) {
+    if (!x.f32 || A.bv || A.tag != 1)
+        throw Error(PMC_ERR_INTERNAL, "Lanczos operator passes: shared values, fp32-stored input, the solver's operator");
+}
+int spmm_z_dot(hipStream_t st, int nb, const SellView& A, zvec x, double* dot_partial) {
+    check_lanczos_pass(A, x);
+    const LanczosUpdate none{};
+    return spmm_t<float>(st, nb, A, x.as<float>(), nullptr, false, dot_partial, x.as<float>(), 1, &none);
+}
+void spmm_z_update(hipStream_t st, int nb, const SellView& A, zvec x, const LanczosUpdate& lz, double* v, bool v_zero) {
+    check_lanczos_pass(A, x);
+    if (!lz.c0 || !lz.c1 || !lz.c2 || !lz.v1 || !lz.y32 || !v)
+        throw Error(PMC_ERR_INTERNAL, "Lanczos update pass: operand missing");
+    spmm_t<float>(st, nb, A, x.as<float>(), v, false, nullptr, nullptr, v_zero ? 3 : 2, &lz);
 }
 
 void residual_restrict8(hipStream_t st, int nb, const SellView& A, const double* r, const double* x, double* out,
@@ -3329,6 +3403,12 @@
     return dot_partial ? (int)g.x : 0;
 }
 
+void copy_r32(hipStream_t st, int nb, int n, const double* in, double* out, float* out32) {
+    if (n == 0) return;
+    PMC_DISPATCH_NB(nb, { copy_r32_kernel<NB><<<grid_dot(n, nb), kBlock, 0, st>>>(flat_count(n, nb), in, out, out32); });
+    check_launch();
+}
+
 int wdot(hipStream_t st, int nb, int n, const double* w, const double* x, double* partial) {
     const dim3 g = grid_dot(n, nb);
     PMC_DISPATCH_NB(nb, { wdot_kernel<NB><<<g, kBlock, 0, st>>>(flat_count(n, nb), w, x, partial, nb); });
diff --git a/parelagmc_amd/csrc/kernels.hpp b/parelagmc_amd/csrc/kernels.hpp
--- a/parelagmc_amd/csrc/kernels.hpp
+++ b/parelagmc_amd/csrc/kernels.hpp
@@ -94,6 +94,15 @@
 int spmm(hipStream_t st, int nb, const SellView& A, const double* x, double* y, bool accumulate,
           double* dot_partial, const double* dot_with);
 int spmm_z(hipStream_t st, int nb, const SellView& A, zvec x, double* y, double* dot_partial, zvec dot_with);
+struct LanczosUpdate {
+    const double* __restrict__ c0 = nullptr;
+    const double* __restrict__ c1 = nullptr;
+    const double* __restrict__ c2 = nullptr;
+    const double* __restrict__ v1 = nullptr;
+    float* __restrict__ y32 = nullptr;
+};
+int spmm_z_dot(hipStream_t st, int nb, const SellView& A, zvec x, double* dot_partial);
+void spmm_z_update(hipStream_t st, int nb, const SellView& A, zvec x, const LanczosUpdate& lz, double* v, bool v_zero);
 void residual_restrict8(hipStream_t st, int nb, const SellView& A, const double* r, const double* x, double* out,
                         double* coarse);
 void residual(hipStream_t st, int nb, const SellView& A, const double* r, const double* x, double* out);
@@ -143,6 +152,7 @@
 int wdot(hipStream_t st, int nb, int n, const double* w, const double* x, double* partial);
 int dot_z(hipStream_t st, int nb, int n, const double* a, zvec b, double* partial);
 int convert_z(hipStream_t st, int nb, int n, const double* in, zvec out, const double* r, double* dot_partial);
+void copy_r32(hipStream_t st, int nb, int n, const double* in, double* out, float* out32);
 void reduce_final(hipStream_t st, int nb, int nblocks, const double* partial, double* out);
 void lincomb3(hipStream_t st, int nb, int n, const double* c0, const double* a, const double* c1, const double* b,
               const double* c2, double* y, float* y32 = nullptr);
diff --git a/parelagmc_amd/csrc/sampler.hip b/parelagmc_amd/csrc/sampler.hip
--- a/parelagmc_amd/csrc/sampler.hip
+++ b/parelagmc_amd/csrc/sampler.hip
@@ -626,6 +626,14 @@
     A.apply_z = [Av](const Lanes& L, int nb_, zvec x, double* y, double* partial, double*) {
         return k::DotParts{partial, k::spmm_z(L.main, nb_, Av, x, y, partial, x)};
     };
+    if (hybrid && !Av.bv) {
+        A.apply_z_dot = [Av](const Lanes& L, int nb_, zvec x, double* partial, double*) {
+            return k::DotParts{partial, k::spmm_z_dot(L.main, nb_, Av, x, partial)};
+        };
+        A.apply_z_update = [Av](const Lanes& L, int nb_, zvec x, const k::LanczosUpdate& lz, double* v, bool v_zero) {
+            k::spmm_z_update(L.main, nb_, Av, x, lz, v, v_zero);
+        };
+    }
     PrecFn prec = preconditioner(level, nb, degM, mgp, mg_l0);
     work.want_r32 = hybrid && opts.precond_storage != PMC_STORAGE_FP64 && mgp->top_reads_r32(mg_l0, nb);
     if (const char* e = lab_env("PMC_R32")) work.want_r32 = work.want_r32 && atoi(e) != 0;
diff --git a/parelagmc_amd/csrc/solver.hip b/parelagmc_amd/csrc/solver.hip
--- a/parelagmc_amd/csrc/solver.hip
+++ b/parelagmc_amd/csrc/solver.hip
@@ -410,10 +410,11 @@
     return h;
 }
 
-void MinresWork::ensure(int n, int nb, bool z32) {
+void MinresWork::ensure(int n, int nb, bool z32, bool need_q) {
     const size_t need = (size_t)n * nb;
     v0.ensure(need); v1.ensure(need); u0.ensure(need, z32); u1.ensure(need, z32);
-    w0.ensure(need); w1.ensure(need); q.ensure(need);
+    w0.ensure(need); w1.ensure(need);
+    if (need_q) q.ensure(need);
     partial.ensure((size_t)2 * dot_capacity(n, nb) * nb);
     partial_op.ensure((size_t)2 * dot_capacity(n, nb) * nb);
     if (!state.p) state.alloc(1);
@@ -513,6 +514,17 @@
     return (int)std::min<size_t>(std::max<size_t>(fit, 9) - 1, (size_t)k::kWxWindow);
 }
 
+static std::atomic<uint64_t> g_fused_solves{0};
+uint64_t fused_lanczos_solve_count() { return g_fused_solves.load(std::memory_order_relaxed); }
+
+static bool fused_lanczos_on() {
+    static const bool v = [] {
+        const char* e = lab_env("PMC_FUSED_LANCZOS");
+        return !e || atoi(e) != 0;
+    }();
+    return v;
+}
+
 static bool late_wx() {
     static const bool v = [] {
         const char* e = lab_env("PMC_LATE_WX");
@@ -531,7 +543,14 @@
                                               Ctx::contexts_on_device(ctx.device) == 1);
     const Lanes L = ctx.lanes(split);
     const bool z32 = o.precond_storage != PMC_STORAGE_FP64;
-    w.ensure(n, nb, z32);
+    const int every = o.check_every > 0 ? o.check_every : 1;
+    const bool graphs = hint.key != 0 && o.use_graph != 0 && every == 2;
+    const bool late = L.split && !graphs && A.n0 > 0 && A.n0 < n && late_wx();
+    const bool r32 = w.want_r32 && z32;
+    const bool timing = w.op_timer.on && !(hint.key != 0 && o.use_graph != 0);
+    const bool fused = A.apply_z_dot && A.apply_z_update && !graphs && !late && r32 && !timing && fused_lanczos_on();
+    w.ensure(n, nb, z32, !fused);
+    if (r32) w.r32.ensure(len);
     k::MinresState* S = w.state.p;
     double* v0 = w.v0.p; double* v1 = w.v1.p; zvec u0 = w.u0.v(z32); zvec u1 = w.u1.v(z32);
     double* w0 = w.w0.p; double* w1 = w.w1.p; double* q = w.q.p;
@@ -540,10 +559,8 @@
     if (!A.apply_z || (!zero_guess && !A.apply)) throw Error(PMC_ERR_INTERNAL, "minres: operator closures missing");
     if (x_row0 < 0 || x_nrows < 0 || (!x_rows && x_row0 + x_nrows > n))
         throw Error(PMC_ERR_INTERNAL, "minres: bad solution row range");
+    if (fused) g_fused_solves.fetch_add(1, std::memory_order_relaxed);
     const size_t xoff = (size_t)x_row0 * nb;
-    const int every = o.check_every > 0 ? o.check_every : 1;
-    const bool graphs = hint.key != 0 && o.use_graph != 0 && every == 2;
-    const bool late = L.split && !graphs && A.n0 > 0 && A.n0 < n && late_wx();
     const bool defer = !graphs && !late && !x_rows && wx_defer_on();
     if (zero_guess) {
         if (defer) {
@@ -552,23 +569,20 @@
         } else {
             k::fill(st, x_rows ? (size_t)x_nrows * nb : len, x, 0.0);
         }
-        k::copy(st, len, b, v1);
+        if (r32) k::copy_r32(st, nb, n, b, v1, w.r32.p);
+        else k::copy(st, len, b, v1);
     } else {
         A.apply(L, nb, x, v1, nullptr, nullptr);
         axpby(st, len, 1.0, b, -1.0, v1);
+        if (r32) k::convert_z(st, nb, n, v1, zvec(reinterpret_cast<double*>(w.r32.p), true), nullptr, nullptr);
     }
     const size_t seg2 = (size_t)dot_capacity(n, nb) * nb;
-    const bool r32 = w.want_r32 && z32;
-    if (r32) {
-        w.r32.ensure(len);
-        k::convert_z(st, nb, n, v1, zvec(reinterpret_cast<double*>(w.r32.p), true), nullptr, nullptr);
-        w.r32_valid = true;
-    }
+    w.r32_valid = r32;
     k::DotParts dp = prec(L, nb, v1, u1, w.partial.p, w.partial.p + seg2);
     if (dp.total() == 0) dp = k::DotParts{w.partial.p, k::dot_z(st, nb, n, v1, u1, w.partial.p)};
     const int window = defer ? wx_window(ctx.device, len * (z32 ? sizeof(float) : sizeof(double))) : 1;
     k::minres_init(st, nb, S, dp, o.rel_tol, o.abs_tol, window);
-    k::fill(st, len, v0, 0.0);
+    if (!fused) k::fill(st, len, v0, 0.0);
     if (!defer) {
         k::fill(st, len, w0, 0.0);
         k::fill(st, len, w1, 0.0);
@@ -596,9 +610,12 @@
         w.u2.ensure(len, z32);
         u2 = w.u2.v(z32);
     }
-    const bool timing = w.op_timer.on && !(hint.key != 0 && o.use_graph != 0);
     k::DotParts dp_op;
     auto apply_op = [&](zvec u) {
+        if (fused) {
+            dp_op = A.apply_z_dot(L, nb, u, w.partial_op.p, w.partial_op.p + seg2);
+            return;
+        }
         if (timing) w.op_timer.begin(st);
         dp_op = A.apply_z(L, nb, u, q, w.partial_op.p, w.partial_op.p + seg2);
         if (timing) w.op_timer.end(st);
@@ -612,8 +629,16 @@
         if (pend.u) wx(s, pend.u, pend.w0, pend.w1);
         pend.u = zvec();
     };
+    int it = 0;
     auto iteration = [&](zvec u0_, zvec u1_, double* v0_, double* v1_, double* w0_, double* w1_, bool last) {
-        if (late) {
+        if (fused) {
+            k::LanczosUpdate lz;
+            lz.c0 = cV0; lz.c1 = cV1; lz.c2 = cV2;
+            lz.v1 = v1_;
+            lz.y32 = w.r32.p;
+            A.apply_z_update(L, nb, u1_, lz, v0_, it == 1);
+            w.r32_valid = true;
+        } else if (late) {
             const size_t off = (size_t)A.n0 * nb;
             L.fork();
             k::lincomb3(L.aux, nb, A.n0, cV0, q, cV1, v1_, cV2, v0_);
@@ -639,7 +664,6 @@
         iteration(u0, u1, v0, v1, w0, w1, false);
         iteration(u1, u0, v1, v0, w1, w0, false);
     };
-    int it = 0;
     int n_active = poll();
     const uint64_t hint_key = hint.key ? hash_mix(hint.key, zero_guess ? 1 : 2) : 0;
     int first_poll = 0;
diff --git a/parelagmc_amd/csrc/solver.hpp b/parelagmc_amd/csrc/solver.hpp
--- a/parelagmc_amd/csrc/solver.hpp
+++ b/parelagmc_amd/csrc/solver.hpp
@@ -121,6 +121,8 @@
                               double* dot_partial2)> apply;
     std::function<k::DotParts(const Lanes& L, int nb, zvec x, double* y, double* dot_partial,
                               double* dot_partial2)> apply_z;
+    std::function<k::DotParts(const Lanes& L, int nb, zvec x, double* dot_partial, double* dot_partial2)> apply_z_dot;
+    std::function<void(const Lanes& L, int nb, zvec x, const k::LanczosUpdate& lz, double* v, bool v_zero)> apply_z_update;
 };
 using PrecFn = std::function<k::DotParts(const Lanes& L, int nb, const double* r, zvec z, double* dot_partial,
                                          double* dot_partial2)>;
@@ -194,8 +196,10 @@
     MinresWork(const MinresWork&) = delete;
     MinresWork& operator=(const MinresWork&) = delete;
     ~MinresWork();
-    void ensure(int n, int nb, bool z32);
-};
+    void ensure(int n, int nb, bool z32, bool need_q = true);
+};
+
+uint64_t fused_lanczos_solve_count();
 
 struct MinresResult {
     pmc_stats col[kMaxBatch];
```

Measured after the change: 4396 samples/s, median of 6. 6.4% higher.
